# jopohl/urh

Hardware: NVIDIA H100
Metric: MSamples/s IQ demod+digitize (complex64) (higher is better)
Workload: dtype f32

## Files before the change

### urh_b200/csrc/dense_f32.cuh

```cuda
#pragma once
#include "dense.cuh"

struct SrcQad {
    static constexpr bool BINARY = false;
    template <typename T> __device__ __forceinline__ static int cls(T s, const UrhClassify& C, float) { return urh_classify((float)s, C); }
    template <typename T> __device__ __forceinline__ static void bits(T, const UrhClassify&, float, bool& nz, bool& ab) { nz = false; ab = false; }
    template <typename T> __device__ __forceinline__ static bool above(T, float) { return false; }
};
struct SrcQad2 {
    static constexpr bool BINARY = true;
    template <typename T> __device__ __forceinline__ static int cls(T s, const UrhClassify& C, float thr0) {
        const int c = ((float)s <= thr0) ? 0 : 1;
        return ((float)s == C.noise_value) ? -1 : c;
    }
    template <typename T> __device__ __forceinline__ static void bits(T s, const UrhClassify& C, float thr0, bool& nz, bool& ab) {
        nz = (float)s == C.noise_value;
        ab = !((float)s <= thr0) && !nz;
    }
    template <typename T> __device__ __forceinline__ static bool above(T s, float thr0) { return !((float)s <= thr0); }
};
struct SrcAbove {
    static constexpr bool BINARY = true;
    template <typename T> __device__ __forceinline__ static int cls(T s, const UrhClassify&, float thr0) { return (s > (T)thr0) ? 1 : 0; }
    template <typename T> __device__ __forceinline__ static void bits(T s, const UrhClassify&, float thr0, bool& nz, bool& ab) { nz = false; ab = s > (T)thr0; }
    template <typename T> __device__ __forceinline__ static bool above(T s, float thr0) { return s > (T)thr0; }
};
struct SrcCenter {
    static constexpr bool BINARY = true;
    template <typename T> __device__ __forceinline__ static int cls(T s, const UrhClassify&, float thr0) { return (s <= (T)thr0) ? 0 : 1; }
    template <typename T> __device__ __forceinline__ static void bits(T s, const UrhClassify&, float thr0, bool& nz, bool& ab) { nz = false; ab = !(s <= (T)thr0); }
    template <typename T> __device__ __forceinline__ static bool above(T s, float thr0) { return !(s <= (T)thr0); }
};

struct UrhSpec {
    const float* tg;
    float* margin;
    int64_t lo, hi;
    unsigned int* redone;
};

template <typename T> struct UrhVec2;
template <> struct UrhVec2<float> { typedef float2 type; };
template <> struct UrhVec2<double> { typedef double2 type; };

template <typename SRC, typename T>
__global__ void __launch_bounds__(URH_WARPS_PER_BLOCK * 32)
k_dense_f32(const T* __restrict__ x, int64_t n, int vec_in, const __grid_constant__ UrhClassify cls, int tol,
            UrhTileSummary* __restrict__ tiles, uint32_t* __restrict__ staging, int stage_cap,
            int16_t* __restrict__ init_cls, int cls_of_zero, const float* __restrict__ d_thr0 = nullptr,
            const UrhTileStats* __restrict__ tile_stats = nullptr, const UrhSpec spec = UrhSpec{}) {
    const float thr0 = d_thr0 ? *d_thr0 : cls.thr[0];
    if (d_thr0) cls_of_zero = (0.0f <= thr0) ? 0 : 1;
    const int lane = threadIdx.x & 31;
    const int64_t tile = (int64_t)blockIdx.x * URH_WARPS_PER_BLOCK + (threadIdx.x >> 5);
    const int64_t tile_start = tile * URH_TILE;
    if (tile_start >= n) return;
    const int tile_len = (int)((n - tile_start) < URH_TILE ? (n - tile_start) : URH_TILE);
    const int iters = (tile_len + 63) >> 6;
    if (tile_stats && tile_stats[tile].all_noise) {
        if (lane == 0) {
            UrhTileSummary s;
            s.first_cls = -1; s.last_cls = -1; s.head_len = tile_len; s.tail_len = tile_len; s.ncand = 0;
            tiles[tile] = s;
            if (tile_start == 0 && init_cls) *init_cls = (int16_t)-1;
        }
        return;
    }
    if (tile >= spec.lo && tile < spec.hi) {
        if (spec.margin[tile] > fabsf(__fsub_rn(thr0, *spec.tg))) return;
        if (lane == 0) atomicAdd(spec.redone, 1u);
    }
    UrhRunTracker rt;
    rt.init(tol, staging + tile * (int64_t)stage_cap);
    if (vec_in && tile_len == URH_TILE) {
        typedef typename UrhVec2<T>::type V;
        const V* p = (const V*)(x + tile_start) + lane;
        constexpr int ITERS = URH_TILE / 64;
        const bool no_noise = SRC::BINARY && tile_stats && cls.noise_value <= -4.0f && tile_stats[tile].cnt == URH_TILE;
        V cur[4], nxt[4];
#pragma unroll
        for (int j = 0; j < 4; j++) cur[j] = __ldg(p + j * 32);
        if (tile_start == 0 && lane == 0 && init_cls) *init_cls = (int16_t)(((float)cur[0].x == cls.noise_value) ? -1 : cls_of_zero);
        if (SRC::BINARY) {
            UrhTileResolve tr;
            tr.init();
#pragma unroll 1
            for (int it = 0; it < ITERS; it += 4) {
                if (it + 4 < ITERS) {
#pragma unroll
                    for (int j = 0; j < 4; j++) nxt[j] = __ldg(p + (it + 4 + j) * 32);
                }
                if (no_noise) {
#pragma unroll
                    for (int j = 0; j < 4; j++)
                        tr.keep(it + j, 0u, __ballot_sync(URH_FULL_MASK, SRC::template above<T>(cur[j].x, thr0)), 0u,
                                __ballot_sync(URH_FULL_MASK, SRC::template above<T>(cur[j].y, thr0)), lane);
                } else {
#pragma unroll
                    for (int j = 0; j < 4; j++) {
                        bool nx, ax, ny, ay;
                        SRC::template bits<T>(cur[j].x, cls, thr0, nx, ax);
                        SRC::template bits<T>(cur[j].y, cls, thr0, ny, ay);
                        tr.keep(it + j, __ballot_sync(URH_FULL_MASK, nx), __ballot_sync(URH_FULL_MASK, ax), __ballot_sync(URH_FULL_MASK, ny),
                                __ballot_sync(URH_FULL_MASK, ay), lane);
                    }
                }
#pragma unroll
                for (int j = 0; j < 4; j++) cur[j] = nxt[j];
            }
            tr.finish(tol, staging + tile * (int64_t)stage_cap, tiles + tile, lane);
            return;
        }
#pragma unroll 1
        for (int it = 0; it < ITERS; it += 4) {
            if (it + 4 < ITERS) {
#pragma unroll
                for (int j = 0; j < 4; j++) nxt[j] = __ldg(p + (it + 4 + j) * 32);
            }
#pragma unroll
            for (int j = 0; j < 4; j++)
                rt.feed(it + j, SRC::template cls<T>(cur[j].x, cls, thr0), SRC::template cls<T>(cur[j].y, cls, thr0), true, true, lane);
#pragma unroll
            for (int j = 0; j < 4; j++) cur[j] = nxt[j];
        }
        rt.finish(tile_len, tiles + tile, lane);
        return;
    }
    for (int it = 0; it < iters; it += 2) {
        T a0 = 0, a1 = 0, b0 = 0, b1 = 0;
        const int64_t pa = tile_start + (int64_t)it * 64 + 2 * lane;
        const int64_t pb = pa + 64;
        if (vec_in && pa + 1 < n) {
            const typename UrhVec2<T>::type v = __ldg((const typename UrhVec2<T>::type*)(x + pa));
            a0 = v.x; a1 = v.y;
        } else {
            if (pa < n) a0 = __ldg(x + pa);
            if (pa + 1 < n) a1 = __ldg(x + pa + 1);
        }
        const bool has_b = it + 1 < iters;
        if (has_b) {
            if (vec_in && pb + 1 < n) {
                const typename UrhVec2<T>::type v = __ldg((const typename UrhVec2<T>::type*)(x + pb));
                b0 = v.x; b1 = v.y;
            } else {
                if (pb < n) b0 = __ldg(x + pb);
                if (pb + 1 < n) b1 = __ldg(x + pb + 1);
            }
        }
        if (pa == 0 && init_cls) *init_cls = (int16_t)(((float)a0 == cls.noise_value) ? -1 : cls_of_zero);
        rt.feed(it, SRC::template cls<T>(a0, cls, thr0), SRC::template cls<T>(a1, cls, thr0), pa < n, pa + 1 < n, lane);
        if (has_b) rt.feed(it + 1, SRC::template cls<T>(b0, cls, thr0), SRC::template cls<T>(b1, cls, thr0), pb < n, pb + 1 < n, lane);
    }
    rt.finish(tile_len, tiles + tile, lane);
}
```

### urh_b200/csrc/digitize.cu

```cuda
#include "dense.cuh"
#include "scan.cuh"
#include "sparse.cuh"
#ifndef URH_FAST_MIN_BLOCKS
#define URH_FAST_MIN_BLOCKS 4
#endif
#include "fsk_fast.cuh"
#include "dense_f32.cuh"

#include <math.h>
#include <stdlib.h>


template <int DT, int MOD, bool DIGITIZE>
__device__ __forceinline__ void dense_iq_tile(const void* __restrict__ iq, int64_t n, const UrhDemodParams& dp, float* __restrict__ qad_out,
                                              int vec_in, int vec_out, const UrhClassify& cls, int tol, UrhTileSummary* __restrict__ tiles,
                                              uint32_t* __restrict__ staging, int stage_cap, int16_t* __restrict__ init_cls, int cls_of_zero,
                                              int64_t tile, int has_halo, UrhTileStats* __restrict__ tile_stats, const UrhFine& fine,
                                              unsigned int* s_fine, unsigned int* g_fine) {
    const int lane = threadIdx.x & 31;
    const int64_t tile_start = tile * URH_TILE;
    const int tile_len = (int)((n - tile_start) < URH_TILE ? (n - tile_start) : URH_TILE);
    const int iters = (tile_len + 63) >> 6;

    UrhRunTracker rt;
    if (DIGITIZE) rt.init(tol, staging + tile * (int64_t)stage_cap);
    UrhStatAcc acc;
    acc.init();

    float cA = 0.0f, cB = 0.0f;
    if (MOD == URH_MOD_FSK && (tile_start > 0 || has_halo) && lane == 0) {
        typedef typename UrhElem<DT>::type E;
        const E* pp = (const E*)iq + 2 * (tile_start - 1);
        const UrhFskTerms t = urh_fsk_terms((float)pp[0], (float)pp[1]);
        cA = t.A; cB = t.B;
    }

    UrhPair cur = urh_load_pair<DT>(iq, tile_start + 2 * lane, n, vec_in != 0);
    for (int it = 0; it < iters; it++) {
        const int64_t pos0 = tile_start + (int64_t)it * 64 + 2 * lane;
        UrhPair nxt;
        if (it + 1 < iters) nxt = urh_load_pair<DT>(iq, pos0 + 64, n, vec_in != 0);

        const float m0 = __fadd_rn(__fmul_rn(cur.r0, cur.r0), __fmul_rn(cur.i0, cur.i0));
        const float m1 = __fadd_rn(__fmul_rn(cur.r1, cur.r1), __fmul_rn(cur.i1, cur.i1));
        float s0 = dp.noise_value, s1 = dp.noise_value;
        if (MOD == URH_MOD_FSK) {
            const UrhFskTerms t0 = urh_fsk_terms(cur.r0, cur.i0);
            const UrhFskTerms t1 = urh_fsk_terms(cur.r1, cur.i1);
            float pA = __shfl_up_sync(URH_FULL_MASK, t1.A, 1);
            float pB = __shfl_up_sync(URH_FULL_MASK, t1.B, 1);
            if (lane == 0) { pA = cA; pB = cB; }
            cA = __shfl_sync(URH_FULL_MASK, t1.A, 31);
            cB = __shfl_sync(URH_FULL_MASK, t1.B, 31);
            if (!(m0 <= dp.noise_sqrd)) s0 = urh_fsk_angle(pA, pB, t0.C, t0.D);
            if (!(m1 <= dp.noise_sqrd)) s1 = urh_fsk_angle(t0.A, t0.B, t1.C, t1.D);
        } else if (MOD == URH_MOD_ASK) {
            if (!(m0 <= dp.noise_sqrd)) s0 = __fdiv_rn(__fsqrt_rn(m0), dp.max_mag);
            if (!(m1 <= dp.noise_sqrd)) s1 = __fdiv_rn(__fsqrt_rn(m1), dp.max_mag);
        }
        if (pos0 == 0 && !has_halo) s0 = dp.noise_value;

        const bool v0 = pos0 < n, v1 = pos0 + 1 < n;
        if (tile_stats) {
            if (v0) { acc.add(s0); acc.all_noise = acc.all_noise && (s0 == dp.noise_value); }
            if (v1) { acc.add(s1); acc.all_noise = acc.all_noise && (s1 == dp.noise_value); }
            if (s_fine) {
                if (v0) urh_fine_add(s0, fine, s_fine, g_fine);
                if (v1) urh_fine_add(s1, fine, s_fine, g_fine);
            }
        }
        if (qad_out) {
            if (v1 && vec_out) urh_stg_f2(qad_out + pos0, s0, s1);
            else {
                if (v0) qad_out[pos0] = s0;
                if (v1) qad_out[pos0 + 1] = s1;
            }
        }
        if (DIGITIZE) {
            const int c0 = urh_classify(s0, cls), c1 = urh_classify(s1, cls);
            if (pos0 == 0) *init_cls = (int16_t)((s0 == cls.noise_value) ? -1 : cls_of_zero);
            rt.feed(it, c0, c1, v0, v1, lane);
        }
        cur = nxt;
    }
    if (tile_stats) acc.store(tile_stats + tile, lane);
    if (DIGITIZE) rt.finish(tile_len, tiles + tile, lane);
}

template <int DT, int MOD, bool DIGITIZE>
__global__ void __launch_bounds__(URH_WARPS_PER_BLOCK * 32)
k_dense_iq(const void* __restrict__ iq, int64_t n, UrhDemodParams dp, float* __restrict__ qad_out, int vec_in,
           int vec_out, const __grid_constant__ UrhClassify cls, int tol, UrhTileSummary* __restrict__ tiles,
           uint32_t* __restrict__ staging, int stage_cap, int16_t* __restrict__ init_cls, int cls_of_zero,
           int64_t tile_begin, int64_t tile_count, int has_halo, UrhTileStats* __restrict__ tile_stats, const UrhFine fine) {
    extern __shared__ unsigned int s_fine[];
    const int64_t tile_rel = (int64_t)blockIdx.x * URH_WARPS_PER_BLOCK + (threadIdx.x >> 5);
    const int64_t block_tile0 = tile_begin + (int64_t)blockIdx.x * URH_WARPS_PER_BLOCK;
    if (fine.gh) urh_fine_zero(s_fine);
    if (tile_rel < tile_count && (tile_begin + tile_rel) * URH_TILE < n)
        dense_iq_tile<DT, MOD, DIGITIZE>(iq, n, dp, qad_out, vec_in, vec_out, cls, tol, tiles, staging, stage_cap, init_cls, cls_of_zero,
                                    tile_begin + tile_rel, has_halo, tile_stats, fine,
                                    fine.gh ? s_fine : nullptr, fine.gh ? urh_fine_row(fine, tile_begin + tile_rel, block_tile0) : nullptr);
    if (fine.gh) urh_fine_flush(fine, s_fine, block_tile0);
}

template <int DT, bool DIGITIZE, bool WRITE, bool STATS>
__global__ void __launch_bounds__(URH_WARPS_PER_BLOCK * 32, URH_FAST_MIN_BLOCKS)
k_fsk_fast(const void* __restrict__ iq, int64_t n, UrhDemodParams dp, float* __restrict__ qad_out, float thr0,
           float cls_noise, int tol, UrhTileSummary* __restrict__ tiles, uint32_t* __restrict__ staging, int stage_cap,
           int64_t tile_begin, int64_t tile_count, UrhTileStats* __restrict__ tile_stats, const UrhFine fine) {
    extern __shared__ unsigned int s_fine[];
    const bool fine_on = STATS && fine.gh;
    const int lane = threadIdx.x & 31;
    const int64_t tile_rel = (int64_t)blockIdx.x * URH_WARPS_PER_BLOCK + (threadIdx.x >> 5);
    const int64_t block_tile0 = tile_begin + (int64_t)blockIdx.x * URH_WARPS_PER_BLOCK;
    if (fine_on) urh_fine_zero(s_fine);
    if (tile_rel < tile_count) {
        const int64_t tile = tile_begin + tile_rel;
        UrhRunTracker rt;
        if (DIGITIZE) rt.init(tol, staging + tile * (int64_t)stage_cap);
        UrhOne one;
        one.p = dp.one;
        one.m = dp.mone;
        urh_fsk_full_tile<DT, DIGITIZE, WRITE, STATS>(iq, n, tile * URH_TILE, dp, qad_out, thr0, cls_noise, rt, lane, one,
                                                      STATS ? tile_stats + tile : nullptr, 0u, DIGITIZE ? tiles + tile : nullptr, fine,
                                                      fine_on ? s_fine : nullptr, fine_on ? urh_fine_row(fine, tile, block_tile0) : nullptr);
    }
    if (fine_on) urh_fine_flush(fine, s_fine, block_tile0);
}

#define URH_FSK_FIFO 3
template <int DT, bool DIGITIZE, bool WRITE, bool STATS>
__global__ void __launch_bounds__(URH_WARPS_PER_BLOCK * 32, (DT == URH_DT_F32) ? 5 : 4)
k_fsk_fifo(const void* __restrict__ iq, int64_t n, UrhDemodParams dp, float* __restrict__ qad_out, float thr0,
           float cls_noise, int tol, UrhTileSummary* __restrict__ tiles, uint32_t* __restrict__ staging, int stage_cap,
           int64_t tile_begin, int64_t tile_count, UrhTileStats* __restrict__ tile_stats, const UrhFine fine,
           const float* __restrict__ d_thr0 = nullptr, float* __restrict__ margin = nullptr) {
    __shared__ __align__(16) unsigned char s_fifo[URH_WARPS_PER_BLOCK][URH_FSK_FIFO + 1][64 * 2 * sizeof(typename UrhElem<DT>::type)];
    extern __shared__ unsigned int s_fine[];
    const bool fine_on = STATS && fine.gh;
    if (DIGITIZE && STATS) thr0 = *d_thr0;
    const int lane = threadIdx.x & 31;
    const int64_t tile_rel = (int64_t)blockIdx.x * URH_WARPS_PER_BLOCK + (threadIdx.x >> 5);
    const int64_t block_tile0 = tile_begin + (int64_t)blockIdx.x * URH_WARPS_PER_BLOCK;
    if (fine_on) urh_fine_zero(s_fine);
    if (tile_rel < tile_count) {
        const int64_t tile = tile_begin + tile_rel;
        UrhRunTracker rt;
        if (DIGITIZE) rt.init(tol, staging + tile * (int64_t)stage_cap);
        UrhOne one;
        one.p = dp.one;
        one.m = dp.mone;
        const uint32_t fifo = (uint32_t)__cvta_generic_to_shared(&s_fifo[threadIdx.x >> 5][0][0]);
        urh_fsk_full_tile<DT, DIGITIZE, WRITE, STATS, URH_FSK_FIFO>(iq, n, tile * URH_TILE, dp, qad_out, thr0, cls_noise, rt, lane, one,
                                                                    STATS ? tile_stats + tile : nullptr, fifo,
                                                                    DIGITIZE ? tiles + tile : nullptr, fine, fine_on ? s_fine : nullptr,
                                                                    fine_on ? urh_fine_row(fine, tile, block_tile0) : nullptr,
                                                                    (DIGITIZE && STATS) ? margin + tile : nullptr);
    }
    if (fine_on) urh_fine_flush(fine, s_fine, block_tile0);
}

#define URH_GUESS_SAMPLES 16384
#define URH_GUESS_BINS 128
#define URH_GUESS_THREADS 1024
__global__ void __launch_bounds__(URH_GUESS_THREADS) k_speculate_guess(const float2* __restrict__ iq, int64_t n, float noise_sqrd, int forced,
                                                                      float forced_tg, float* __restrict__ d_tg, unsigned int* __restrict__ redone) {
    constexpr int PER = URH_GUESS_SAMPLES / URH_GUESS_THREADS;
    __shared__ unsigned int s_hist[URH_GUESS_BINS];
    __shared__ float s_mn[32], s_mx[32];
    if (forced) {
        if (threadIdx.x == 0) { *d_tg = forced_tg; *redone = 0u; }
        return;
    }
    for (int b = threadIdx.x; b < URH_GUESS_BINS; b += blockDim.x) s_hist[b] = 0u;
    float v[PER];
    float mn = INFINITY, mx = -INFINITY;
#pragma unroll
    for (int k = 0; k < PER; k++) {
        const int64_t i = 1 + (int64_t)(k * URH_GUESS_THREADS + threadIdx.x) * (n - 1) / URH_GUESS_SAMPLES;
        const float2 p = iq[i - 1], c = iq[i];
        v[k] = NAN;
        if (!(c.x * c.x + c.y * c.y <= noise_sqrd)) {
            v[k] = atan2f(p.x * c.y - p.y * c.x, p.x * c.x + p.y * c.y);
            mn = fminf(mn, v[k]);
            mx = fmaxf(mx, v[k]);
        }
    }
    for (int off = 16; off > 0; off >>= 1) {
        mn = fminf(mn, __shfl_xor_sync(URH_FULL_MASK, mn, off));
        mx = fmaxf(mx, __shfl_xor_sync(URH_FULL_MASK, mx, off));
    }
    if ((threadIdx.x & 31) == 0) { s_mn[threadIdx.x >> 5] = mn; s_mx[threadIdx.x >> 5] = mx; }
    __syncthreads();
    mn = INFINITY; mx = -INFINITY;
    for (int w = 0; w < URH_GUESS_THREADS / 32; w++) { mn = fminf(mn, s_mn[w]); mx = fmaxf(mx, s_mx[w]); }
    const float width = (mx - mn) / URH_GUESS_BINS;
    if (width > 0.0f) {
#pragma unroll
        for (int k = 0; k < PER; k++)
            if (!isnan(v[k])) atomicAdd(&s_hist[min((int)((v[k] - mn) / width), URH_GUESS_BINS - 1)], 1u);
    }
    __syncthreads();
    if (threadIdx.x != 0) return;
    *redone = 0u;
    if (!(mn <= mx)) { *d_tg = 0.0f; return; }
    if (!(width > 0.0f)) { *d_tg = mn; return; }
    constexpr int WINDOW = (int)(0.05 * URH_GUESS_BINS) + 1;
    int top[2] = {-1, -1};
    for (int b = 0; b < URH_GUESS_BINS; b++) {
        const unsigned int y = s_hist[b];
        bool peak = y > 0u;
        for (int d = 1; d < WINDOW && peak; d++)
            peak = y > (b + d < URH_GUESS_BINS ? s_hist[b + d] : 0u) && y > (b - d >= 0 ? s_hist[b - d] : 0u);
        if (!peak) continue;
        if (top[0] < 0 || y > s_hist[top[0]]) { top[1] = top[0]; top[0] = b; }
        else if (top[1] < 0 || y > s_hist[top[1]]) top[1] = b;
    }
    if (top[0] < 0) *d_tg = 0.5f * (mn + mx);
    else if (top[1] < 0) *d_tg = mn + ((float)top[0] + 0.5f) * width;
    else *d_tg = mn + (0.5f * (float)(top[0] + top[1]) + 0.5f) * width;
}


extern "C" int urh_get_center_thresholds(float center, float spacing, int modulation_order, float* h_out) {
    const int n = modulation_order / 2;
    for (int i = 0; i < n; i++) {
        volatile float t = (float)(n - (i + 1)) * spacing;
        h_out[i] = center - t;
    }
    for (int i = n; i < modulation_order - 1; i++) {
        volatile float t = (float)(i + 1 - n) * spacing;
        h_out[i] = center + t;
    }
    return URH_OK;
}

static int fill_classify(urh_ctx* ctx, UrhClassify* C, int mod_type, float center, uint8_t bits_per_symbol,
                         float spacing) {
    if (bits_per_symbol > 8) URH_FAIL(ctx, URH_ERR_INVALID, "bits_per_symbol %d > 8 not supported", (int)bits_per_symbol);
    memset(C, 0, sizeof(*C));
    C->noise_value = urh_noise_value(mod_type);
    C->order = 1 << bits_per_symbol;
    if (C->order > 1) urh_get_center_thresholds(center, spacing, C->order, C->thr);
    return URH_OK;
}

static int host_classify(float s, const UrhClassify& C) {
    int c = C.order - 1;
    for (int k = 0; k < C.order - 1; k++)
        if (s <= C.thr[k]) { c = k; break; }
    return c;
}

static float max_magnitude_for(int dtype) {
    switch (dtype) {
        case URH_DT_I8: return (float)sqrt(127.0 * 127.0 + 128.0 * 128.0);
        case URH_DT_U8: return (float)sqrt(255.0 * 255.0);
        case URH_DT_I16: return (float)sqrt(32768.0 * 32768.0 + 32767.0 * 32767.0);
        case URH_DT_U16: return (float)sqrt(65535.0 * 65535.0);
        default: return (float)sqrt(2.0);
    }
}

static bool iq_vec_aligned(const void* p, int dtype) { return ((uintptr_t)p % (2 * (size_t)urh_iq_bytes(dtype))) == 0; }

template <int DT, int MOD, bool DIG>
static int launch_dense_iq_t(urh_ctx* ctx, const void* d_iq, int64_t n, const UrhDemodParams& dp, float* d_qad,
                             const UrhClassify& cls, int tol, UrhTileSummary* tiles, uint32_t* staging,
                             int stage_cap, int16_t* init_cls, int cls_of_zero, int has_halo = 0,
                             UrhTileStats* tile_stats = nullptr, int64_t tile_lo = 0, int64_t tile_hi = -1,
                             const UrhFine& fine = UrhFine{}, UrhSpec* spec = nullptr) {
    const int64_t ntiles = urh_div_up(n, URH_TILE);
    const size_t fine_smem = fine.gh ? (size_t)URH_FINE_NB * sizeof(unsigned int) : 0;
    if (tile_hi < 0 || tile_hi > ntiles) tile_hi = ntiles;
    const int vec_in = iq_vec_aligned(d_iq, DT) ? 1 : 0;
    const int vec_out = (d_qad && ((uintptr_t)d_qad % 8) == 0) ? 1 : 0;
    const int threads = URH_WARPS_PER_BLOCK * 32;
    auto generic = [&](int64_t begin, int64_t end) -> int {
        begin = begin < tile_lo ? tile_lo : begin;
        end = end > tile_hi ? tile_hi : end;
        const int64_t count = end - begin;
        if (count <= 0) return URH_OK;
        URH_LAUNCH(ctx, (k_dense_iq<DT, MOD, DIG>), (unsigned)urh_div_up(count, URH_WARPS_PER_BLOCK), threads, fine_smem, d_iq, n, dp,
                   d_qad, vec_in, vec_out, cls, tol, tiles, staging, stage_cap, init_cls, cls_of_zero, begin, count, has_halo,
                   tile_stats, fine);
        return URH_OK;
    };
    const int64_t nfull = n / URH_TILE;
    const bool fast = MOD == URH_MOD_FSK && vec_in && (!d_qad || vec_out) && (!DIG || cls.order == 2) && nfull > 1;
    URH_PROF_BEGIN(ctx);
    if (fast) {
        const int64_t fb = tile_lo > 1 ? tile_lo : 1, fe = tile_hi < nfull ? tile_hi : nfull;
        if (fe > fb) {
            const unsigned grid = (unsigned)urh_div_up(fe - fb, URH_WARPS_PER_BLOCK);
            static const bool fifo = getenv("URH_B200_FSK_NO_FIFO") == nullptr;
            const bool ff = fifo;
            bool speculated = false;
            if constexpr (DT == URH_DT_F32 && MOD == URH_MOD_FSK && !DIG) {
                if (spec && ff && tile_stats && d_qad) {
                    URH_LAUNCH(ctx, (k_fsk_fifo<DT, true, true, true>), grid, threads, fine_smem, d_iq, n, dp, d_qad, 0.0f, dp.noise_value,
                               tol, tiles, staging, stage_cap, fb, fe - fb, tile_stats, fine, (const float*)spec->tg, spec->margin);
                    spec->lo = fb;
                    spec->hi = fe;
                    speculated = true;
                }
            }
            if (speculated) {
            } else if (tile_stats && d_qad && !DIG) {
                if (ff) URH_LAUNCH(ctx, (k_fsk_fifo<DT, false, true, true>), grid, threads, fine_smem, d_iq, n, dp, d_qad, cls.thr[0], cls.noise_value,
                                   tol, tiles, staging, stage_cap, fb, fe - fb, tile_stats, fine);
                else URH_LAUNCH(ctx, (k_fsk_fast<DT, false, true, true>), grid, threads, fine_smem, d_iq, n, dp, d_qad, cls.thr[0], cls.noise_value,
                                tol, tiles, staging, stage_cap, fb, fe - fb, tile_stats, fine);
            } else if (d_qad) {
                if (ff) URH_LAUNCH(ctx, (k_fsk_fifo<DT, DIG, true, false>), grid, threads, 0, d_iq, n, dp, d_qad, cls.thr[0], cls.noise_value, tol,
                                   tiles, staging, stage_cap, fb, fe - fb, nullptr, UrhFine{});
                else URH_LAUNCH(ctx, (k_fsk_fast<DT, DIG, true, false>), grid, threads, 0, d_iq, n, dp, d_qad, cls.thr[0], cls.noise_value, tol,
                                tiles, staging, stage_cap, fb, fe - fb, nullptr, UrhFine{});
            } else {
                if (ff) URH_LAUNCH(ctx, (k_fsk_fifo<DT, DIG, false, false>), grid, threads, 0, d_iq, n, dp, d_qad, cls.thr[0], cls.noise_value, tol,
                                   tiles, staging, stage_cap, fb, fe - fb, nullptr, UrhFine{});
                else URH_LAUNCH(ctx, (k_fsk_fast<DT, DIG, false, false>), grid, threads, 0, d_iq, n, dp, d_qad, cls.thr[0], cls.noise_value, tol,
                                tiles, staging, stage_cap, fb, fe - fb, nullptr, UrhFine{});
            }
        }
        URH_CHECK(generic(0, 1));
        URH_CHECK(generic(nfull, ntiles));
    } else {
        URH_CHECK(generic(0, ntiles));
    }
    URH_PROF_END(ctx);
    return URH_OK;
}

template <int MOD, bool DIG>
static int launch_dense_iq_m(urh_ctx* ctx, int dtype, const void* d_iq, int64_t n, const UrhDemodParams& dp,
                             float* d_qad, const UrhClassify& cls, int tol, UrhTileSummary* tiles,
                             uint32_t* staging, int stage_cap, int16_t* init_cls, int cls_of_zero, int has_halo = 0,
                             UrhTileStats* tile_stats = nullptr, int64_t tile_lo = 0, int64_t tile_hi = -1,
                             const UrhFine& fine = UrhFine{}, UrhSpec* spec = nullptr) {
    switch (dtype) {
        case URH_DT_I8: return launch_dense_iq_t<URH_DT_I8, MOD, DIG>(ctx, d_iq, n, dp, d_qad, cls, tol, tiles, staging, stage_cap, init_cls, cls_of_zero, has_halo, tile_stats, tile_lo, tile_hi, fine);
        case URH_DT_U8: return launch_dense_iq_t<URH_DT_U8, MOD, DIG>(ctx, d_iq, n, dp, d_qad, cls, tol, tiles, staging, stage_cap, init_cls, cls_of_zero, has_halo, tile_stats, tile_lo, tile_hi, fine);
        case URH_DT_I16: return launch_dense_iq_t<URH_DT_I16, MOD, DIG>(ctx, d_iq, n, dp, d_qad, cls, tol, tiles, staging, stage_cap, init_cls, cls_of_zero, has_halo, tile_stats, tile_lo, tile_hi, fine);
        case URH_DT_U16: return launch_dense_iq_t<URH_DT_U16, MOD, DIG>(ctx, d_iq, n, dp, d_qad, cls, tol, tiles, staging, stage_cap, init_cls, cls_of_zero, has_halo, tile_stats, tile_lo, tile_hi, fine);
        case URH_DT_F32: return launch_dense_iq_t<URH_DT_F32, MOD, DIG>(ctx, d_iq, n, dp, d_qad, cls, tol, tiles, staging, stage_cap, init_cls, cls_of_zero, has_halo, tile_stats, tile_lo, tile_hi, fine, spec);
        default: URH_FAIL(ctx, URH_ERR_DTYPE, "Unsupported dtype");
    }
}

int urh_costas_demod(urh_ctx* ctx, const void* d_iq, int dtype, int64_t n, float noise_sqrd, int loop_order,
                     float bandwidth, float* d_out);

static UrhDemodParams make_demod_params(float noise_mag, int mod_type, int dtype) {
    UrhDemodParams dp;
    volatile float nm = noise_mag;
    volatile float sq = nm * nm;
    dp.noise_sqrd = sq;
    dp.noise_value = urh_noise_value(mod_type);
    dp.max_mag = max_magnitude_for(dtype);
    dp.one = 1.0f;
    dp.mone = -1.0f;
    return dp;
}

extern "C" int urh_afp_demod(urh_ctx* ctx, const void* d_iq, int dtype, int64_t n, float noise_mag, int mod_type,
                             int mod_order, float costas_loop_bandwidth, float* d_out) {
    if (n < 0) URH_FAIL(ctx, URH_ERR_INVALID, "negative length");
    if (urh_iq_bytes(dtype) == 0) URH_FAIL(ctx, URH_ERR_DTYPE, "Unsupported dtype");
    if (n == 0) return URH_OK;
    if (n <= 2 || (mod_type != URH_MOD_ASK && mod_type != URH_MOD_FSK && mod_type != URH_MOD_PSK)) {
        URH_CUDA(ctx, cudaMemsetAsync(d_out, 0, (size_t)n * sizeof(float), ctx->stream));
        if (n > 2) {
            const float nv = urh_noise_value(mod_type);
            URH_CUDA(ctx, cudaMemcpyAsync(d_out, &nv, sizeof(float), cudaMemcpyHostToDevice, ctx->stream));
            URH_CUDA(ctx, cudaStreamSynchronize(ctx->stream));
        }
        return URH_OK;
    }
    const UrhDemodParams dp = make_demod_params(noise_mag, mod_type, dtype);
    if (mod_type == URH_MOD_PSK) return urh_costas_demod(ctx, d_iq, dtype, n, dp.noise_sqrd, mod_order, costas_loop_bandwidth, d_out);
    UrhClassify cls;
    memset(&cls, 0, sizeof(cls));
    if (mod_type == URH_MOD_ASK)
        return launch_dense_iq_m<URH_MOD_ASK, false>(ctx, dtype, d_iq, n, dp, d_out, cls, 0, nullptr, nullptr, 0, nullptr, 0);
    return launch_dense_iq_m<URH_MOD_FSK, false>(ctx, dtype, d_iq, n, dp, d_out, cls, 0, nullptr, nullptr, 0, nullptr, 0);
}

int urh_center_tiles_begin(urh_ctx* ctx, const float* d_x, const UrhTileStats* ts, int64_t n, int64_t* h_total);

extern "C" int urh_afp_demod_tiles(urh_ctx* ctx, const void* d_iq, int dtype, int64_t n, float noise_mag, int mod_type,
                                   float* d_qad_out, int halo, int64_t* h_kept) {
    if (n <= 2 || (mod_type != URH_MOD_ASK && mod_type != URH_MOD_FSK) || !d_qad_out)
        URH_FAIL(ctx, URH_ERR_INVALID, "urh_afp_demod_tiles: ASK/FSK, n > 2 and a qad buffer are required");
    if (urh_iq_bytes(dtype) == 0) URH_FAIL(ctx, URH_ERR_DTYPE, "Unsupported dtype");
    urh_arena_reset(ctx);
    const UrhDemodParams dp = make_demod_params(noise_mag, mod_type, dtype);
    UrhClassify cls;
    memset(&cls, 0, sizeof(cls));
    const int64_t ntiles = urh_div_up(n, URH_TILE);
    UrhTileStats* ts;
    URH_CHECK(urh_arena(ctx, (size_t)ntiles, &ts));
    if (mod_type == URH_MOD_ASK)
        URH_CHECK((launch_dense_iq_m<URH_MOD_ASK, false>(ctx, dtype, d_iq, n, dp, d_qad_out, cls, 0, nullptr, nullptr, 0, nullptr, 0, halo, ts)));
    else
        URH_CHECK((launch_dense_iq_m<URH_MOD_FSK, false>(ctx, dtype, d_iq, n, dp, d_qad_out, cls, 0, nullptr, nullptr, 0, nullptr, 0, halo, ts)));
    return urh_center_tiles_begin(ctx, d_qad_out, ts, n, h_kept);
}

int urh_finish_local(urh_ctx* ctx, int64_t n, int tol, bool is_ask, uint32_t sps, const UrhTileSummary* tiles, const uint32_t* staging,
                     int stage_cap, const int16_t* d_init, int64_t* k);
int urh_finish_shard(urh_ctx* ctx, int64_t n, int tol, bool is_ask, uint32_t sps, const UrhTileSummary* tiles, const uint32_t* staging,
                     int stage_cap, const int16_t* d_init, int64_t global_offset, int64_t n_total, int64_t* k);

static int digitize_finish(urh_ctx* ctx, int64_t n, int tol, bool is_ask, uint32_t sps, UrhTileSummary* tiles,
                           uint32_t* staging, int stage_cap, int16_t* d_init, int64_t* k) {
    if (getenv("URH_B200_OLD_FINISH")) {
        UrhCandidates cand;
        URH_CHECK(urh_collect_candidates(ctx, n, tol, tiles, staging, stage_cap, &cand));
        return urh_pulses_from_candidates(ctx, n, tol, is_ask, sps, cand, d_init, k);
    }
    return urh_finish_local(ctx, n, tol, is_ask, sps, tiles, staging, stage_cap, d_init, k);
}

static int stage_cap_for(int tol) { return URH_TILE / (tol + 1) + 2; }

extern "C" int urh_grab_pulse_lens(urh_ctx* ctx, const float* d_qad, int64_t n, float center, uint16_t tolerance,
                                   int mod_type, uint32_t samples_per_symbol, uint8_t bits_per_symbol,
                                   float center_spacing, int64_t* k) {
    if (!k) return URH_ERR_INVALID;
    *k = 0;
    ctx->pulses_k = 0;
    if (n < 0) URH_FAIL(ctx, URH_ERR_INVALID, "negative length");
    if (n == 0) return URH_OK;
    urh_arena_reset(ctx);
    UrhClassify cls;
    URH_CHECK(fill_classify(ctx, &cls, mod_type, center, bits_per_symbol, center_spacing));
    const int tol = tolerance;
    const int64_t ntiles = urh_div_up(n, URH_TILE);
    const int cap = stage_cap_for(tol);
    UrhTileSummary* tiles;
    uint32_t* staging;
    int16_t* d_init;
    URH_CHECK(urh_arena(ctx, (size_t)ntiles, &tiles));
    URH_CHECK(urh_arena(ctx, (size_t)ntiles * cap, &staging));
    URH_CHECK(urh_arena(ctx, 8, &d_init));
    const unsigned grid = (unsigned)urh_div_up(ntiles, URH_WARPS_PER_BLOCK);
    const int vec_in = (((uintptr_t)d_qad % 8) == 0) ? 1 : 0;
    URH_PROF_BEGIN(ctx);
    if (cls.order == 2)
        URH_LAUNCH(ctx, (k_dense_f32<SrcQad2, float>), grid, URH_WARPS_PER_BLOCK * 32, 0, d_qad, n, vec_in, cls, tol, tiles,
                   staging, cap, d_init, host_classify(0.0f, cls));
    else
        URH_LAUNCH(ctx, (k_dense_f32<SrcQad, float>), grid, URH_WARPS_PER_BLOCK * 32, 0, d_qad, n, vec_in, cls, tol, tiles,
                   staging, cap, d_init, host_classify(0.0f, cls));
    URH_PROF_END(ctx);
    return digitize_finish(ctx, n, tol, mod_type == URH_MOD_ASK, samples_per_symbol, tiles, staging, cap, d_init, k);
}

extern "C" int urh_demod_digitize(urh_ctx* ctx, const void* d_iq, int dtype, int64_t n, float noise_mag,
                                  int mod_type, float center, uint16_t tolerance, uint32_t samples_per_symbol,
                                  uint8_t bits_per_symbol, float center_spacing, float* d_qad_out, int64_t* k) {
    if (!k) return URH_ERR_INVALID;
    *k = 0;
    ctx->pulses_k = 0;
    if (n < 0) URH_FAIL(ctx, URH_ERR_INVALID, "negative length");
    if (urh_iq_bytes(dtype) == 0) URH_FAIL(ctx, URH_ERR_DTYPE, "Unsupported dtype");
    if (n == 0) return URH_OK;
    if (n <= 2 || (mod_type != URH_MOD_ASK && mod_type != URH_MOD_FSK)) {
        float* q = d_qad_out;
        if (!q) URH_CUDA(ctx, cudaMalloc((void**)&q, (size_t)n * sizeof(float)));
        int rc = urh_afp_demod(ctx, d_iq, dtype, n, noise_mag, mod_type, 1 << bits_per_symbol, 0.1f, q);
        if (rc == URH_OK)
            rc = urh_grab_pulse_lens(ctx, q, n, center, tolerance, mod_type, samples_per_symbol, bits_per_symbol,
                                     center_spacing, k);
        if (!d_qad_out) {
            cudaStreamSynchronize(ctx->stream);
            cudaFree(q);
        }
        return rc;
    }
    urh_arena_reset(ctx);
    UrhClassify cls;
    URH_CHECK(fill_classify(ctx, &cls, mod_type, center, bits_per_symbol, center_spacing));
    const UrhDemodParams dp = make_demod_params(noise_mag, mod_type, dtype);
    const int tol = tolerance;
    const int64_t ntiles = urh_div_up(n, URH_TILE);
    const int cap = stage_cap_for(tol);
    UrhTileSummary* tiles;
    uint32_t* staging;
    int16_t* d_init;
    URH_CHECK(urh_arena(ctx, (size_t)ntiles, &tiles));
    URH_CHECK(urh_arena(ctx, (size_t)ntiles * cap, &staging));
    URH_CHECK(urh_arena(ctx, 8, &d_init));
    const int c0 = host_classify(0.0f, cls);
    if (mod_type == URH_MOD_ASK)
        URH_CHECK((launch_dense_iq_m<URH_MOD_ASK, true>(ctx, dtype, d_iq, n, dp, d_qad_out, cls, tol, tiles, staging, cap, d_init, c0)));
    else
        URH_CHECK((launch_dense_iq_m<URH_MOD_FSK, true>(ctx, dtype, d_iq, n, dp, d_qad_out, cls, tol, tiles, staging, cap, d_init, c0)));
    return digitize_finish(ctx, n, tol, mod_type == URH_MOD_ASK, samples_per_symbol, tiles, staging, cap, d_init, k);
}

extern "C" int urh_shard_dense(urh_ctx* ctx, const void* d_iq, int dtype, int64_t n, int has_halo, float noise_mag, int mod_type,
                               float center, uint16_t tolerance, uint8_t bits_per_symbol, float center_spacing,
                               float* d_qad_out, int64_t* h_summary) {
    if (n <= 0) URH_FAIL(ctx, URH_ERR_INVALID, "empty shard");
    if (mod_type != URH_MOD_ASK && mod_type != URH_MOD_FSK) URH_FAIL(ctx, URH_ERR_INVALID, "sharded path: ASK / FSK only (PSK is a serial recurrence)");
    if (urh_iq_bytes(dtype) == 0) URH_FAIL(ctx, URH_ERR_DTYPE, "Unsupported dtype");
    urh_arena_reset(ctx);
    UrhClassify cls;
    URH_CHECK(fill_classify(ctx, &cls, mod_type, center, bits_per_symbol, center_spacing));
    const UrhDemodParams dp = make_demod_params(noise_mag, mod_type, dtype);
    const int tol = tolerance;
    const int64_t ntiles = urh_div_up(n, URH_TILE);
    const int cap = stage_cap_for(tol);
    UrhTileSummary* tiles;
    uint32_t* staging;
    int16_t* d_init;
    URH_CHECK(urh_arena(ctx, (size_t)ntiles, &tiles));
    URH_CHECK(urh_arena(ctx, (size_t)ntiles * cap, &staging));
    URH_CHECK(urh_arena(ctx, 8, &d_init));
    URH_CUDA(ctx, cudaMemsetAsync(d_init, 0, 16, ctx->stream));
    const int c0 = host_classify(0.0f, cls);
    if (mod_type == URH_MOD_ASK)
        URH_CHECK((launch_dense_iq_m<URH_MOD_ASK, true>(ctx, dtype, d_iq, n, dp, d_qad_out, cls, tol, tiles, staging, cap, d_init, c0, has_halo)));
    else
        URH_CHECK((launch_dense_iq_m<URH_MOD_FSK, true>(ctx, dtype, d_iq, n, dp, d_qad_out, cls, tol, tiles, staging, cap, d_init, c0, has_halo)));
    ctx->shard_tiles = tiles;
    ctx->shard_staging = staging;
    ctx->shard_cap = cap;
    ctx->shard_n = n;
    ctx->shard_tol = tol;
    URH_CHECK(urh_shard_run_total(ctx, n, tiles, h_summary));
    int16_t init16 = 0;
    URH_CUDA(ctx, cudaMemcpyAsync(&init16, d_init, sizeof(int16_t), cudaMemcpyDeviceToHost, ctx->stream));
    URH_CUDA(ctx, cudaStreamSynchronize(ctx->stream));
    h_summary[3] = init16;
    return URH_OK;
}

extern "C" int urh_shard_dense_qad(urh_ctx* ctx, const float* d_qad, int64_t n, int mod_type, float center, uint16_t tolerance,
                                   uint8_t bits_per_symbol, float center_spacing, int64_t* h_summary) {
    if (n <= 0) URH_FAIL(ctx, URH_ERR_INVALID, "empty shard");
    urh_arena_reset(ctx);
    UrhClassify cls;
    URH_CHECK(fill_classify(ctx, &cls, mod_type, center, bits_per_symbol, center_spacing));
    const int tol = tolerance;
    const int64_t ntiles = urh_div_up(n, URH_TILE);
    const int cap = stage_cap_for(tol);
    UrhTileSummary* tiles;
    uint32_t* staging;
    int16_t* d_init;
    URH_CHECK(urh_arena(ctx, (size_t)ntiles, &tiles));
    URH_CHECK(urh_arena(ctx, (size_t)ntiles * cap, &staging));
    URH_CHECK(urh_arena(ctx, 8, &d_init));
    URH_CUDA(ctx, cudaMemsetAsync(d_init, 0, 16, ctx->stream));
    const int vec_in = (((uintptr_t)d_qad % 8) == 0) ? 1 : 0;
    URH_PROF_BEGIN(ctx);
    const unsigned grid = (unsigned)urh_div_up(ntiles, URH_WARPS_PER_BLOCK);
    if (cls.order == 2)
        URH_LAUNCH(ctx, (k_dense_f32<SrcQad2, float>), grid, URH_WARPS_PER_BLOCK * 32, 0, d_qad, n, vec_in, cls, tol, tiles, staging, cap,
                   d_init, host_classify(0.0f, cls));
    else
        URH_LAUNCH(ctx, (k_dense_f32<SrcQad, float>), grid, URH_WARPS_PER_BLOCK * 32, 0, d_qad, n, vec_in, cls, tol, tiles, staging, cap,
                   d_init, host_classify(0.0f, cls));
    URH_PROF_END(ctx);
    ctx->shard_tiles = tiles;
    ctx->shard_staging = staging;
    ctx->shard_cap = cap;
    ctx->shard_n = n;
    ctx->shard_tol = tol;
    URH_CHECK(urh_shard_run_total(ctx, n, tiles, h_summary));
    int16_t init16 = 0;
    URH_CUDA(ctx, cudaMemcpyAsync(&init16, d_init, sizeof(int16_t), cudaMemcpyDeviceToHost, ctx->stream));
    URH_CUDA(ctx, cudaStreamSynchronize(ctx->stream));
    h_summary[3] = init16;
    return URH_OK;
}

int urh_finish_chunk(urh_ctx* ctx, int64_t n, int tol, bool is_ask, uint32_t sps, const UrhTileSummary* tiles, const uint32_t* staging,
                     int stage_cap, const int16_t* d_init, UrhChain* chain, int64_t global_offset, int64_t n_total, int64_t row_base,
                     int64_t rows_cap, int64_t* k);

#define URH_STREAM_MAX_RING 8
#define URH_STREAM_PAD 256
enum { URH_OP_UPLOAD = 0, URH_OP_COMPUTE = 1, URH_OP_DOWNLOAD = 2 };

static int64_t stream_chunk_samples(int64_t n, int64_t cs) {
    if (cs <= 0) cs = (int64_t)1 << 24;
    cs -= cs % URH_TILE;
    if (cs < URH_TILE) cs = URH_TILE;
    const int64_t whole = urh_div_up(n > 0 ? n : 1, URH_TILE) * URH_TILE;
    return cs < whole ? cs : whole;
}
static int64_t rows_bound(int64_t n, int tol) { return n / (tol + 1) + 3; }

extern "C" int urh_stream_schedule(int64_t n, int64_t chunk_samples, int ring, int flags, int64_t* h_ops, int64_t cap, int64_t* count) {
    if (!count || n < 0 || ring < 2 || ring > URH_STREAM_MAX_RING) return URH_ERR_INVALID;
    const int64_t cs = stream_chunk_samples(n, chunk_samples);
    const int64_t chunks = urh_div_up(n, cs);
    const bool up = flags & URH_STREAM_UPLOAD, down = flags & URH_STREAM_DOWNLOAD, halo = flags & URH_STREAM_HALO;
    int64_t k = 0;
    auto emit = [&](int64_t kind, int64_t c) {
        if (h_ops && k < cap) {
            int64_t* o = h_ops + 6 * k;
            o[0] = kind; o[1] = c; o[2] = c % ring; o[3] = c * cs; o[4] = (c + 1) * cs < n ? (c + 1) * cs : n;
            o[5] = (kind == URH_OP_UPLOAD && halo && c > 0) ? 1 : 0;
        }
        k++;
    };
    if (up)
        for (int64_t c = 0; c < ring - 1 && c < chunks; c++) emit(URH_OP_UPLOAD, c);
    for (int64_t c = 0; c < chunks; c++) {
        if (up && c + ring - 1 < chunks) emit(URH_OP_UPLOAD, c + ring - 1);
        emit(URH_OP_COMPUTE, c);
        if (down) emit(URH_OP_DOWNLOAD, c);
    }
    *count = k;
    return (h_ops && k > cap) ? URH_ERR_INVALID : URH_OK;
}

struct StreamSizes {
    int64_t cs;
    int64_t src_slot;
    int64_t qad_slot;
    int64_t ring_bytes;
    int64_t arena;
    int64_t scan_items;
    int64_t rows_chunk;
};
static int64_t r256(int64_t b) { return (b + 255) & ~(int64_t)255; }
static int64_t finish_arena_bytes(int64_t tiles, int64_t rows_cap, bool ask) {
    return r256(tiles * (int64_t)sizeof(RunCarry)) + 2 * r256(tiles * 4) + 2 * r256(tiles * 8) + r256((32 + 8) * 8) +
           (ask ? r256(rows_cap * 16) : 0);
}
static int psk_order_of(int entry) { return (entry & URH_STREAM_PSK) ? ((entry & URH_STREAM_PSK4) ? 4 : 2) : 0; }
static int psk_entry_flags(int mod_order) { return URH_STREAM_PSK | (mod_order >= 4 ? URH_STREAM_PSK4 : 0); }

static StreamSizes stream_sizes(int64_t n, int dtype, int tol, int64_t chunk_samples, int ring, int entry) {
    StreamSizes z;
    const int kind = entry & 0xf;
    const int psk = psk_order_of(entry);
    const bool resident = entry & URH_STREAM_RESIDENT;
    const int64_t ntiles = urh_div_up(n, URH_TILE);
    z.cs = resident ? ntiles * URH_TILE : stream_chunk_samples(n, chunk_samples);
    const int64_t ct = z.cs / URH_TILE;
    const int64_t cap = stage_cap_for(tol);
    const bool iq = kind != URH_STREAM_ENTRY_GRAB_PULSE_LENS;
    const bool digitize = kind != URH_STREAM_ENTRY_AFP_DEMOD;
    z.rows_chunk = rows_bound(z.cs, tol);
    if (resident) {
        z.src_slot = iq ? n * urh_iq_bytes(dtype) : n * 4;
        z.qad_slot = (kind == URH_STREAM_ENTRY_GRAB_PULSE_LENS) ? 0 : n * 4;
        z.ring_bytes = r256(z.src_slot) + r256(z.qad_slot);
    } else {
        z.src_slot = (kind == URH_STREAM_ENTRY_GRAB_PULSE_LENS && (entry & URH_STREAM_QAD_ON_DEVICE)) ? 0
                     : URH_STREAM_PAD + z.cs * (iq ? urh_iq_bytes(dtype) : 4);
        const bool qad_ring = kind == URH_STREAM_ENTRY_AFP_DEMOD ||
                              (kind == URH_STREAM_ENTRY_DEMOD_DIGITIZE && ((entry & URH_STREAM_QAD_OUT) || psk));
        z.qad_slot = qad_ring ? z.cs * 4 : 0;
        z.ring_bytes = ring * (r256(z.src_slot) + r256(z.qad_slot));
        if (kind == URH_STREAM_ENTRY_DEMOD_CENTER_DIGITIZE) z.ring_bytes += r256(n * 4);
    }
    z.arena = 0;
    z.scan_items = ct > z.rows_chunk ? ct : z.rows_chunk;
    if (digitize) z.arena += r256(ct * (int64_t)sizeof(UrhTileSummary)) + r256(ct * cap * 4) + r256(16) + r256(sizeof(UrhChain)) +
                             finish_arena_bytes(ct, z.rows_chunk, true);
    if (psk && !resident) z.arena += urh_costas_arena_bytes(z.cs, psk) + r256(16) + r256(6 * 8);
    if (kind == URH_STREAM_ENTRY_DEMOD_CENTER_DIGITIZE) {
        z.arena += r256(ntiles * (int64_t)sizeof(UrhTileStats)) + r256((int64_t)URH_FINE_SLABS * URH_FINE_NB * 4) + r256((ntiles + 1) * 8) +
                   ((int64_t)2 << 20);
        if (ntiles > z.scan_items) z.scan_items = ntiles;
    }
    return z;
}

extern "C" int urh_stream_footprint(int64_t n, int dtype, int tolerance, int64_t chunk_samples, int ring, int entry, int64_t rows,
                                    int64_t* bytes) {
    if (!bytes || n < 0 || tolerance < 0 || tolerance > 0xffff || (entry & 0xf) > URH_STREAM_ENTRY_DEMOD_CENTER_DIGITIZE) return URH_ERR_INVALID;
    if (!(entry & URH_STREAM_RESIDENT) && (ring < 2 || ring > URH_STREAM_MAX_RING)) return URH_ERR_INVALID;
    if ((entry & 0xf) != URH_STREAM_ENTRY_GRAB_PULSE_LENS && urh_iq_bytes(dtype) == 0) return URH_ERR_DTYPE;
    if ((entry & URH_STREAM_PSK) && (entry & 0xf) != URH_STREAM_ENTRY_AFP_DEMOD && (entry & 0xf) != URH_STREAM_ENTRY_DEMOD_DIGITIZE)
        return URH_ERR_INVALID;
    const StreamSizes z = stream_sizes(n, dtype, tolerance, chunk_samples, ring, entry);
    const bool digitize = (entry & 0xf) != URH_STREAM_ENTRY_AFP_DEMOD;
    const int64_t r = rows == -2 ? n / 64 + 1024 : (rows < 0 ? rows_bound(n, tolerance) : rows);
    if (entry & URH_STREAM_RESIDENT) {
        const int64_t ntiles = urh_div_up(n, URH_TILE);
        int64_t b = z.ring_bytes + ((int64_t)64 << 20);
        if (digitize)
            b += r256(ntiles * (int64_t)sizeof(UrhTileSummary)) + r256(ntiles * (int64_t)stage_cap_for(tolerance) * 4) +
                 finish_arena_bytes(ntiles, r + r / 4, true) + 16 * (r + r / 4);
        if ((entry & 0xf) == URH_STREAM_ENTRY_DEMOD_CENTER_DIGITIZE)
            b += r256(ntiles * (int64_t)sizeof(UrhTileStats)) + r256((int64_t)URH_FINE_SLABS * URH_FINE_NB * 4) + r256((ntiles + 1) * 8);
        if (psk_order_of(entry)) b += urh_costas_arena_bytes(n, psk_order_of(entry));
        *bytes = b;
        return URH_OK;
    }
    int64_t b = z.ring_bytes;
    b += 2 * z.arena + ((int64_t)64 << 20);
    const int64_t nb = 2 * (z.scan_items / 256 + 1);
    b += 256 + (nb > 8192 ? nb : 8192) * (4 + 2 * 32);
    if (digitize) b += 3 * 16 * (r + z.rows_chunk);
    *bytes = b;
    return URH_OK;
}

extern "C" int urh_stream_stats(urh_ctx* ctx, int64_t* h_out3) {
    h_out3[0] = ctx->stream_free_low;
    h_out3[1] = ctx->stream_chunks;
    h_out3[2] = (int64_t)ctx->arena_peak;
    return URH_OK;
}

struct StreamRing {
    urh_ctx* ctx = nullptr;
    char* mem = nullptr;
    cudaEvent_t ev[3][URH_STREAM_MAX_RING] = {};
    int ring = 0;
    int init(urh_ctx* c, int r, int64_t bytes) {
        ctx = c;
        ring = r;
        ctx->stream_free_low = -1;
        for (int k = 0; k < 3; k++)
            for (int s = 0; s < r; s++) URH_CUDA(ctx, cudaEventCreateWithFlags(&ev[k][s], cudaEventDisableTiming));
        if (bytes > 0) URH_CUDA(ctx, cudaMallocAsync((void**)&mem, (size_t)bytes, ctx->stream));
        URH_CUDA(ctx, cudaEventRecord(ctx->ev_comp[0], ctx->stream));
        URH_CUDA(ctx, cudaStreamWaitEvent(ctx->copy_stream[0], ctx->ev_comp[0], 0));
        URH_CUDA(ctx, cudaStreamWaitEvent(ctx->copy_stream[1], ctx->ev_comp[0], 0));
        return URH_OK;
    }
    ~StreamRing() {
        if (!ctx) return;
        cudaStreamSynchronize(ctx->copy_stream[0]);
        cudaStreamSynchronize(ctx->copy_stream[1]);
        if (mem) cudaFreeAsync(mem, ctx->stream);
        cudaStreamSynchronize(ctx->stream);
        for (int k = 0; k < 3; k++)
            for (int s = 0; s < ring; s++)
                if (ev[k][s]) cudaEventDestroy(ev[k][s]);
    }
};

template <typename F>
static int stream_run(urh_ctx* ctx, int64_t n, int64_t cs, StreamRing& R, const char* h_src, int src_b, bool halo, char* d_src,
                      int64_t src_slot, float* h_qad, float* d_qad, F&& compute, bool qad_resident = false) {
    const int flags = (h_src ? URH_STREAM_UPLOAD : 0) | (h_qad ? URH_STREAM_DOWNLOAD : 0) | (halo ? URH_STREAM_HALO : 0);
    int64_t count = 0;
    URH_CHECK(urh_stream_schedule(n, cs, R.ring, flags, nullptr, 0, &count));
    std::vector<int64_t> ops((size_t)(6 * count));
    URH_CHECK(urh_stream_schedule(n, cs, R.ring, flags, ops.data(), count, &count));
    bool recorded[3][URH_STREAM_MAX_RING] = {};
    ctx->stream_chunks = 0;
    for (int64_t i = 0; i < count; i++) {
        const int64_t* o = &ops[(size_t)(6 * i)];
        const int kind = (int)o[0], s = (int)o[2];
        const int64_t c = o[1], s0 = o[3], s1 = o[4], h = o[5];
        if (kind == URH_OP_UPLOAD) {
            cudaStream_t cp = ctx->copy_stream[0];
            if (recorded[URH_OP_COMPUTE][s]) URH_CUDA(ctx, cudaStreamWaitEvent(cp, R.ev[URH_OP_COMPUTE][s], 0));
            URH_CUDA(ctx, cudaMemcpyAsync(d_src + s * src_slot + URH_STREAM_PAD - h * src_b, h_src + (s0 - h) * src_b,
                                          (size_t)((s1 - s0 + h) * src_b), cudaMemcpyHostToDevice, cp));
            URH_CUDA(ctx, cudaEventRecord(R.ev[URH_OP_UPLOAD][s], cp));
        } else if (kind == URH_OP_COMPUTE) {
            if (h_src) URH_CUDA(ctx, cudaStreamWaitEvent(ctx->stream, R.ev[URH_OP_UPLOAD][s], 0));
            if (h_qad && !qad_resident && recorded[URH_OP_DOWNLOAD][s])
                URH_CUDA(ctx, cudaStreamWaitEvent(ctx->stream, R.ev[URH_OP_DOWNLOAD][s], 0));
            URH_CHECK(compute(c, s0, s1, s));
            URH_CUDA(ctx, cudaEventRecord(R.ev[URH_OP_COMPUTE][s], ctx->stream));
            urh_stream_sample_free(ctx);
            ctx->stream_chunks++;
        } else {
            cudaStream_t cp = ctx->copy_stream[1];
            URH_CUDA(ctx, cudaStreamWaitEvent(cp, R.ev[URH_OP_COMPUTE][s], 0));
            URH_CUDA(ctx, cudaMemcpyAsync(h_qad + s0, d_qad + (qad_resident ? s0 : (int64_t)s * cs), (size_t)(s1 - s0) * sizeof(float),
                                          cudaMemcpyDeviceToHost, cp));
            URH_CUDA(ctx, cudaEventRecord(R.ev[URH_OP_DOWNLOAD][s], cp));
        }
        recorded[kind][s] = true;
    }
    URH_CUDA(ctx, cudaStreamSynchronize(ctx->copy_stream[1]));
    URH_CUDA(ctx, cudaStreamSynchronize(ctx->stream));
    return URH_OK;
}

struct StreamDigitizer {
    UrhTileSummary* tiles;
    uint32_t* staging;
    int16_t* d_init;
    UrhChain* chain;
    int cap, tol;
    bool is_ask;
    uint32_t sps;
    int64_t n, rows, rows_all;
    UrhArenaMark mark;
    int init(urh_ctx* ctx, int64_t n_total, int64_t cs, int tolerance, bool ask, uint32_t samples_per_symbol) {
        n = n_total; tol = tolerance; is_ask = ask; sps = samples_per_symbol; rows = 0;
        cap = stage_cap_for(tol);
        rows_all = rows_bound(n, tol);
        const int64_t ct = cs / URH_TILE;
        URH_CHECK(urh_arena(ctx, (size_t)ct, &tiles));
        URH_CHECK(urh_arena(ctx, (size_t)ct * cap, &staging));
        URH_CHECK(urh_arena(ctx, 8, &d_init));
        URH_CHECK(urh_arena(ctx, 1, &chain));
        URH_CUDA(ctx, cudaMemsetAsync(d_init, 0, 16, ctx->stream));
        mark = urh_arena_mark(ctx);
        return URH_OK;
    }
    int finish(urh_ctx* ctx, int64_t s0, int64_t s1) {
        const int64_t rc = rows_bound(s1 - s0, tol);
        const int64_t need = rows + rc;
        if (need > (int64_t)ctx->pulses_cap_rows) {
            int64_t grow = 2 * (int64_t)ctx->pulses_cap_rows;
            if (grow > rows_all + rc) grow = rows_all + rc;
            URH_CHECK(urh_ensure_pulses_keep(ctx, (size_t)(grow > need ? grow : need), (size_t)rows));
        }
        urh_arena_release(ctx, mark);
        int64_t kc = 0;
        URH_CHECK(urh_finish_chunk(ctx, s1 - s0, tol, is_ask, sps, tiles, staging, cap, d_init, chain, s0, n, rows, rc, &kc));
        urh_stream_sample_free(ctx);
        rows += kc;
        return URH_OK;
    }
};

static int stream_check(urh_ctx* ctx, int64_t n, int ring, int mod_type, int dtype, bool iq);
static int psk_stream_check(urh_ctx* ctx, int64_t n, int ring, int dtype) {
    URH_CHECK(stream_check(ctx, n, ring, URH_MOD_PSK, dtype, false));
    if (n <= 2) URH_FAIL(ctx, URH_ERR_INVALID, "streamed PSK demodulation: n > 2");
    if (urh_iq_bytes(dtype) == 0) URH_FAIL(ctx, URH_ERR_DTYPE, "Unsupported dtype");
    return URH_OK;
}

static int stream_check(urh_ctx* ctx, int64_t n, int ring, int mod_type, int dtype, bool iq) {
    if (n <= 0) URH_FAIL(ctx, URH_ERR_INVALID, "streamed call: empty capture");
    if (ring < 2 || ring > URH_STREAM_MAX_RING) URH_FAIL(ctx, URH_ERR_INVALID, "streamed call: ring of %d slots (2..%d)", ring, URH_STREAM_MAX_RING);
    if (iq && (n <= 2 || (mod_type != URH_MOD_ASK && mod_type != URH_MOD_FSK)))
        URH_FAIL(ctx, URH_ERR_INVALID, "streamed demodulation: ASK/FSK and n > 2 (PSK is a serial recurrence)");
    if (iq && urh_iq_bytes(dtype) == 0) URH_FAIL(ctx, URH_ERR_DTYPE, "Unsupported dtype");
    return URH_OK;
}

template <bool DIG>
static int stream_dense_iq(urh_ctx* ctx, int dtype, int mod_type, const char* d_src, int64_t src_slot, int64_t n, const UrhDemodParams& dp,
                           float* qad_global, const UrhClassify& cls, int tol, StreamDigitizer* dz, int64_t s0, int64_t s1, int s,
                           UrhTileStats* ts = nullptr, const UrhFine& fine = UrhFine{}) {
    const int b = urh_iq_bytes(dtype);
    const void* iq = d_src + s * src_slot + URH_STREAM_PAD - s0 * b;
    const int64_t t0 = s0 / URH_TILE, t1 = urh_div_up(s1, URH_TILE);
    UrhTileSummary* tiles = dz ? dz->tiles - t0 : nullptr;
    uint32_t* staging = dz ? dz->staging - t0 * dz->cap : nullptr;
    const int cap = dz ? dz->cap : 0;
    int16_t* init = dz ? dz->d_init : nullptr;
    const int c0 = DIG ? host_classify(0.0f, cls) : 0;
    if (mod_type == URH_MOD_ASK)
        return launch_dense_iq_m<URH_MOD_ASK, DIG>(ctx, dtype, iq, n, dp, qad_global, cls, tol, tiles, staging, cap, init, c0, 0, ts, t0, t1, fine);
    return launch_dense_iq_m<URH_MOD_FSK, DIG>(ctx, dtype, iq, n, dp, qad_global, cls, tol, tiles, staging, cap, init, c0, 0, ts, t0, t1, fine);
}

static int stream_dense_qad(urh_ctx* ctx, const float* x, int64_t s0, int64_t s1, const UrhClassify& cls, StreamDigitizer& dz,
                            const float* d_thr0 = nullptr, const UrhTileStats* ts = nullptr) {
    const int64_t nc = s1 - s0;
    const unsigned grid = (unsigned)urh_div_up(urh_div_up(nc, URH_TILE), URH_WARPS_PER_BLOCK);
    const int vec_in = (((uintptr_t)x % 8) == 0) ? 1 : 0;
    int16_t* init = s0 == 0 ? dz.d_init : nullptr;
    const int c0 = d_thr0 ? 0 : host_classify(0.0f, cls);
    const UrhTileStats* tsc = ts ? ts + s0 / URH_TILE : nullptr;
    if (cls.order == 2)
        URH_LAUNCH(ctx, (k_dense_f32<SrcQad2, float>), grid, URH_WARPS_PER_BLOCK * 32, 0, x, nc, vec_in, cls, dz.tol, dz.tiles, dz.staging,
                   dz.cap, init, c0, d_thr0, tsc);
    else
        URH_LAUNCH(ctx, (k_dense_f32<SrcQad, float>), grid, URH_WARPS_PER_BLOCK * 32, 0, x, nc, vec_in, cls, dz.tol, dz.tiles, dz.staging,
                   dz.cap, init, c0, d_thr0, tsc);
    return URH_OK;
}

struct CenterPlan;
int urh_center_chain(urh_ctx* ctx, const float* d_qad, int64_t n, const UrhTileStats* ts, int64_t max_size, int rank, int world,
                     const UrhFine* fine, CenterPlan** d_plan_out);
int urh_center_plan_result(urh_ctx* ctx, const CenterPlan* plan, const float** d_centerf, const double** d_center, const int** d_state);
int urh_center_plan_certify_stats(urh_ctx* ctx, const CenterPlan* plan, int64_t* h_dst3);

extern "C" int urh_shard_digitize(urh_ctx* ctx, const void* d_iq, int dtype, const float* d_qad_in, int64_t n, int has_halo,
                                  float noise_mag, int mod_type, float center, uint16_t tolerance, uint32_t samples_per_symbol,
                                  uint8_t bits_per_symbol, float center_spacing, float* d_qad_out, int64_t global_offset,
                                  int64_t n_total, int64_t* k) {
    if (!k) return URH_ERR_INVALID;
    *k = 0;
    ctx->pulses_k = 0;
    if (n <= 0) URH_FAIL(ctx, URH_ERR_INVALID, "empty shard");
    if (mod_type != URH_MOD_ASK && mod_type != URH_MOD_FSK) URH_FAIL(ctx, URH_ERR_INVALID, "sharded path: ASK / FSK only");
    if (!d_qad_in && urh_iq_bytes(dtype) == 0) URH_FAIL(ctx, URH_ERR_DTYPE, "Unsupported dtype");
    if (!ctx->nccl_comm) URH_FAIL(ctx, URH_ERR_INVALID, "NCCL communicator not initialised (urh_nccl_init)");
    urh_arena_reset(ctx);
    UrhClassify cls;
    URH_CHECK(fill_classify(ctx, &cls, mod_type, center, bits_per_symbol, center_spacing));
    const int tol = tolerance;
    const int64_t ntiles = urh_div_up(n, URH_TILE);
    const int cap = stage_cap_for(tol);
    UrhTileSummary* tiles;
    uint32_t* staging;
    int16_t* d_init;
    URH_CHECK(urh_arena(ctx, (size_t)ntiles, &tiles));
    URH_CHECK(urh_arena(ctx, (size_t)ntiles * cap, &staging));
    URH_CHECK(urh_arena(ctx, 8, &d_init));
    URH_CUDA(ctx, cudaMemsetAsync(d_init, 0, 16, ctx->stream));
    const int c0 = host_classify(0.0f, cls);
    if (d_qad_in) {
        const int vec_in = (((uintptr_t)d_qad_in % 8) == 0) ? 1 : 0;
        const unsigned grid = (unsigned)urh_div_up(ntiles, URH_WARPS_PER_BLOCK);
        URH_PROF_BEGIN(ctx);
        if (cls.order == 2)
            URH_LAUNCH(ctx, (k_dense_f32<SrcQad2, float>), grid, URH_WARPS_PER_BLOCK * 32, 0, d_qad_in, n, vec_in, cls, tol, tiles, staging, cap,
                       d_init, c0, (const float*)nullptr);
        else
            URH_LAUNCH(ctx, (k_dense_f32<SrcQad, float>), grid, URH_WARPS_PER_BLOCK * 32, 0, d_qad_in, n, vec_in, cls, tol, tiles, staging, cap,
                       d_init, c0, (const float*)nullptr);
        URH_PROF_END(ctx);
    } else {
        const UrhDemodParams dp = make_demod_params(noise_mag, mod_type, dtype);
        if (mod_type == URH_MOD_ASK)
            URH_CHECK((launch_dense_iq_m<URH_MOD_ASK, true>(ctx, dtype, d_iq, n, dp, d_qad_out, cls, tol, tiles, staging, cap, d_init, c0, has_halo)));
        else
            URH_CHECK((launch_dense_iq_m<URH_MOD_FSK, true>(ctx, dtype, d_iq, n, dp, d_qad_out, cls, tol, tiles, staging, cap, d_init, c0, has_halo)));
    }
    return urh_finish_shard(ctx, n, tol, mod_type == URH_MOD_ASK, samples_per_symbol, tiles, staging, cap, d_init, global_offset, n_total, k);
}

struct StreamCenter {
    int ring;
    int64_t chunk_samples;
    const void* h_iq;
    float* h_qad;
    int64_t* kept;
};
static int demod_center_digitize_impl(urh_ctx* ctx, const void* d_iq, int dtype, int64_t n, int has_halo, float noise_mag, int mod_type,
                                      uint16_t tolerance, uint32_t samples_per_symbol, int64_t max_size, float* d_qad_out, bool sharded,
                                      int64_t global_offset, int64_t n_total, double* center, int* center_state, int64_t* k,
                                      const void* h_iq = nullptr, int64_t chunk_samples = 0, const StreamCenter* sc = nullptr) {
    if (!k || !center || !center_state) return URH_ERR_INVALID;
    *k = 0;
    *center = 0.0;
    *center_state = 0;
    ctx->pulses_k = 0;
    if (n <= 2 || (mod_type != URH_MOD_ASK && mod_type != URH_MOD_FSK) || !d_qad_out)
        URH_FAIL(ctx, URH_ERR_INVALID, "demod_center_digitize: ASK/FSK, n > 2 and a qad buffer are required");
    if (urh_iq_bytes(dtype) == 0) URH_FAIL(ctx, URH_ERR_DTYPE, "Unsupported dtype");
    if (sharded && !ctx->nccl_comm) URH_FAIL(ctx, URH_ERR_INVALID, "NCCL communicator not initialised (urh_nccl_init)");
    urh_arena_reset(ctx);
    URH_TL_RESET(ctx);
    URH_TL_MARK(ctx, "step start");
    const UrhDemodParams dp = make_demod_params(noise_mag, mod_type, dtype);
    UrhClassify cls;
    memset(&cls, 0, sizeof(cls));
    const int64_t ntiles = urh_div_up(n, URH_TILE);
    UrhTileStats* ts;
    URH_CHECK(urh_arena(ctx, (size_t)ntiles, &ts));
    const bool no_certify = getenv("URH_B200_CENTER_NO_CERTIFY") != nullptr;
    UrhFine fine = {};
    if (!sharded && !no_certify) {
        fine.slab_tiles = urh_div_up(ntiles, URH_FINE_SLABS);
        if (fine.slab_tiles < URH_WARPS_PER_BLOCK) fine.slab_tiles = URH_WARPS_PER_BLOCK;
        const int64_t nslabs = urh_div_up(ntiles, fine.slab_tiles);
        URH_CHECK(urh_arena(ctx, (size_t)(nslabs * URH_FINE_NB), &fine.gh));
        URH_CUDA(ctx, cudaMemsetAsync(fine.gh, 0, (size_t)(nslabs * URH_FINE_NB) * sizeof(unsigned int), ctx->stream));
        fine.scale = (mod_type == URH_MOD_FSK) ? 512.0f : 4096.0f;
        fine.off = (mod_type == URH_MOD_FSK) ? 2048.0f : 0.0f;
    }
    const int64_t chunk_tiles = (h_iq && chunk_samples > 0) ? (chunk_samples >= URH_TILE ? chunk_samples / URH_TILE : 1) : ntiles;
    const size_t sample_bytes = (size_t)urh_iq_bytes(dtype);
    StreamRing ring;
    int64_t scs = 0;
    if (sc) {
        const StreamSizes z = stream_sizes(n, dtype, tolerance, sc->chunk_samples, sc->ring, URH_STREAM_ENTRY_DEMOD_CENTER_DIGITIZE);
        scs = z.cs;
        URH_CHECK(ring.init(ctx, sc->ring, sc->ring * r256(z.src_slot)));
        const int64_t slot = r256(z.src_slot);
        URH_CHECK(stream_run(ctx, n, scs, ring, (const char*)sc->h_iq, urh_iq_bytes(dtype), true, ring.mem, slot, sc->h_qad, d_qad_out,
                             [&](int64_t, int64_t s0, int64_t s1, int s) {
                                 return stream_dense_iq<false>(ctx, dtype, mod_type, ring.mem, slot, n, dp, d_qad_out, cls, 0, nullptr, s0, s1, s,
                                                               ts, fine);
                             }, true));
    }
    cls.noise_value = urh_noise_value(mod_type);
    cls.order = 2;
    const int tol = tolerance;
    const int cap = stage_cap_for(tol);
    UrhTileSummary* tiles = nullptr;
    uint32_t* staging = nullptr;
    int16_t* d_init = nullptr;
    if (!sc) {
        URH_CHECK(urh_arena(ctx, (size_t)ntiles, &tiles));
        URH_CHECK(urh_arena(ctx, (size_t)ntiles * cap, &staging));
        URH_CHECK(urh_arena(ctx, 8, &d_init));
    }
    const bool speculate = !sharded && !h_iq && !sc && mod_type == URH_MOD_FSK && dtype == URH_DT_F32 &&
                           getenv("URH_B200_NO_SPECULATE") == nullptr;
    UrhSpec spec = {};
    if (speculate) {
        float* tg;
        URH_CHECK(urh_arena(ctx, 1, &tg));
        URH_CHECK(urh_arena(ctx, 1, &spec.redone));
        URH_CHECK(urh_arena(ctx, (size_t)ntiles, &spec.margin));
        spec.tg = tg;
        const char* forced = getenv("URH_B200_SPECULATE_GUESS");
        URH_LAUNCH(ctx, k_speculate_guess, 1, URH_GUESS_THREADS, 0, (const float2*)d_iq, n, dp.noise_sqrd, forced ? 1 : 0,
                   forced ? strtof(forced, nullptr) : 0.0f, tg, spec.redone);
    }
    int chunk_no = 0;
    for (int64_t t0 = 0; t0 < (sc ? 0 : ntiles); t0 += chunk_tiles, chunk_no++) {
        const int64_t t1 = (t0 + chunk_tiles < ntiles) ? t0 + chunk_tiles : ntiles;
        if (h_iq) {
            const int64_t s0 = t0 * URH_TILE, s1 = (t1 * URH_TILE < n) ? t1 * URH_TILE : n;
            cudaEvent_t ev = ctx->ev_copy[chunk_no & 1];
            URH_CUDA(ctx, cudaMemcpyAsync((char*)d_iq + (size_t)s0 * sample_bytes, (const char*)h_iq + (size_t)s0 * sample_bytes,
                                          (size_t)(s1 - s0) * sample_bytes, cudaMemcpyHostToDevice, ctx->copy_stream[0]));
            URH_CUDA(ctx, cudaEventRecord(ev, ctx->copy_stream[0]));
            URH_CUDA(ctx, cudaStreamWaitEvent(ctx->stream, ev, 0));
        }
        if (mod_type == URH_MOD_ASK)
            URH_CHECK((launch_dense_iq_m<URH_MOD_ASK, false>(ctx, dtype, d_iq, n, dp, d_qad_out, cls, 0, nullptr, nullptr, 0, nullptr, 0, has_halo, ts, t0, t1, fine)));
        else
            URH_CHECK((launch_dense_iq_m<URH_MOD_FSK, false>(ctx, dtype, d_iq, n, dp, d_qad_out, cls, tol, tiles, staging, cap, nullptr, 0, has_halo,
                                                             ts, t0, t1, fine, speculate ? &spec : nullptr)));
    }
    CenterPlan* plan = nullptr;
    URH_CHECK(urh_center_chain(ctx, d_qad_out, n, ts, max_size, sharded ? ctx->nccl_rank : 0, sharded ? ctx->nccl_world : 1,
                               fine.gh ? &fine : nullptr, &plan));
    const float* d_centerf;
    const double* d_center;
    const int* d_state;
    urh_center_plan_result(ctx, plan, &d_centerf, &d_center, &d_state);
    int64_t rows = 0;
    if (sc) {
        URH_CUDA(ctx, cudaMemcpyAsync(ctx->h_mail + 40, d_center, sizeof(double), cudaMemcpyDeviceToHost, ctx->stream));
        URH_CUDA(ctx, cudaMemcpyAsync(ctx->h_mail + 41, d_state, sizeof(int), cudaMemcpyDeviceToHost, ctx->stream));
        URH_CHECK(urh_center_plan_certify_stats(ctx, plan, ctx->h_mail + 42));
        URH_CUDA(ctx, cudaMemcpyAsync(ctx->h_mail + 45, (const int64_t*)ctx->center_prefix + ntiles, sizeof(int64_t), cudaMemcpyDeviceToHost,
                                      ctx->stream));
        URH_CUDA(ctx, cudaStreamSynchronize(ctx->stream));
        int st0 = 0;
        memcpy(&st0, ctx->h_mail + 41, sizeof(int));
        if (st0 == 1) {
            StreamDigitizer dz;
            URH_CHECK(dz.init(ctx, n, scs, tol, mod_type == URH_MOD_ASK, samples_per_symbol));
            for (int64_t s0 = 0; s0 < n; s0 += scs) {
                const int64_t s1 = s0 + scs < n ? s0 + scs : n;
                URH_CHECK(stream_dense_qad(ctx, d_qad_out + s0, s0, s1, cls, dz, d_centerf, ts));
                URH_CHECK(dz.finish(ctx, s0, s1));
            }
            rows = dz.rows;
        }
        *sc->kept = ctx->h_mail[45];
    } else {
        URH_CUDA(ctx, cudaMemsetAsync(d_init, 0, 16, ctx->stream));
        const int vec_in = (((uintptr_t)d_qad_out % 8) == 0) ? 1 : 0;
        URH_LAUNCH(ctx, (k_dense_f32<SrcQad2, float>), (unsigned)urh_div_up(ntiles, URH_WARPS_PER_BLOCK), URH_WARPS_PER_BLOCK * 32, 0,
                   (const float*)d_qad_out, n, vec_in, cls, tol, tiles, staging, cap, d_init, 0, d_centerf, (const UrhTileStats*)ts, spec);
        URH_CUDA(ctx, cudaMemcpyAsync(ctx->h_mail + 40, d_center, sizeof(double), cudaMemcpyDeviceToHost, ctx->stream));
        URH_CUDA(ctx, cudaMemcpyAsync(ctx->h_mail + 41, d_state, sizeof(int), cudaMemcpyDeviceToHost, ctx->stream));
        URH_CHECK(urh_center_plan_certify_stats(ctx, plan, ctx->h_mail + 42));
        ctx->h_mail[46] = 0;
        if (speculate) URH_CUDA(ctx, cudaMemcpyAsync(ctx->h_mail + 46, spec.redone, sizeof(unsigned int), cudaMemcpyDeviceToHost, ctx->stream));
        if (sharded)
            URH_CHECK(urh_finish_shard(ctx, n, tol, mod_type == URH_MOD_ASK, samples_per_symbol, tiles, staging, cap, d_init, global_offset, n_total, &rows));
        else
            URH_CHECK(urh_finish_local(ctx, n, tol, mod_type == URH_MOD_ASK, samples_per_symbol, tiles, staging, cap, d_init, &rows));
    }
    memcpy(center, ctx->h_mail + 40, sizeof(double));
    int st = 0;
    memcpy(&st, ctx->h_mail + 41, sizeof(int));
    *center_state = st;
    ctx->center_cert[0] = ctx->h_mail[42];
    ctx->center_cert[1] = fine.gh ? URH_FINE_NB : 0;
    ctx->center_cert[2] = ctx->h_mail[44];
    const int64_t redone = (spec.hi > spec.lo) ? ctx->h_mail[46] : 0;
    ctx->spec_stats[0] = spec.hi - spec.lo;
    ctx->spec_stats[1] = spec.hi - spec.lo - redone;
    ctx->spec_stats[2] = redone;
    if (st != 1) {
        ctx->pulses_k = 0;
        rows = 0;
    }
    *k = rows;
    return URH_OK;
}

extern "C" int urh_speculate_stats(urh_ctx* ctx, int64_t* h_out3) {
    for (int i = 0; i < 3; i++) h_out3[i] = ctx->spec_stats[i];
    return URH_OK;
}

extern "C" int urh_demod_center_digitize(urh_ctx* ctx, const void* d_iq, int dtype, int64_t n, float noise_mag, int mod_type,
                                         uint16_t tolerance, uint32_t samples_per_symbol, int64_t max_size, float* d_qad_out,
                                         double* center, int* center_state, int64_t* k) {
    return demod_center_digitize_impl(ctx, d_iq, dtype, n, 0, noise_mag, mod_type, tolerance, samples_per_symbol, max_size, d_qad_out, false,
                                      0, n, center, center_state, k);
}

extern "C" int urh_demod_center_digitize_host(urh_ctx* ctx, const void* h_iq, int dtype, int64_t n, float noise_mag, int mod_type,
                                              uint16_t tolerance, uint32_t samples_per_symbol, int64_t max_size, int64_t chunk_samples,
                                              void* d_iq_scratch, float* d_qad_out, double* center, int* center_state, int64_t* k) {
    if (!h_iq || !d_iq_scratch) return URH_ERR_INVALID;
    URH_CUDA(ctx, cudaEventRecord(ctx->ev_comp[0], ctx->stream));
    URH_CUDA(ctx, cudaStreamWaitEvent(ctx->copy_stream[0], ctx->ev_comp[0], 0));
    return demod_center_digitize_impl(ctx, d_iq_scratch, dtype, n, 0, noise_mag, mod_type, tolerance, samples_per_symbol, max_size, d_qad_out,
                                      false, 0, n, center, center_state, k, h_iq, chunk_samples > 0 ? chunk_samples : ((int64_t)1 << 24));
}

extern "C" int urh_shard_demod_center_digitize_host(urh_ctx* ctx, const void* h_iq, int dtype, int64_t n, int has_halo, float noise_mag,
                                                    int mod_type, uint16_t tolerance, uint32_t samples_per_symbol, int64_t max_size,
                                                    int64_t chunk_samples, void* d_iq_scratch, float* d_qad_out, int64_t global_offset,
                                                    int64_t n_total, double* center, int* center_state, int64_t* k) {
    if (!h_iq || !d_iq_scratch) return URH_ERR_INVALID;
    URH_CUDA(ctx, cudaEventRecord(ctx->ev_comp[0], ctx->stream));
    URH_CUDA(ctx, cudaStreamWaitEvent(ctx->copy_stream[0], ctx->ev_comp[0], 0));
    return demod_center_digitize_impl(ctx, d_iq_scratch, dtype, n, has_halo, noise_mag, mod_type, tolerance, samples_per_symbol, max_size,
                                      d_qad_out, true, global_offset, n_total, center, center_state, k, h_iq,
                                      chunk_samples > 0 ? chunk_samples : ((int64_t)1 << 24));
}

extern "C" int urh_shard_demod_center_digitize(urh_ctx* ctx, const void* d_iq, int dtype, int64_t n, int has_halo, float noise_mag,
                                               int mod_type, uint16_t tolerance, uint32_t samples_per_symbol, int64_t max_size,
                                               float* d_qad_out, int64_t global_offset, int64_t n_total, double* center,
                                               int* center_state, int64_t* k) {
    return demod_center_digitize_impl(ctx, d_iq, dtype, n, has_halo, noise_mag, mod_type, tolerance, samples_per_symbol, max_size, d_qad_out,
                                      true, global_offset, n_total, center, center_state, k);
}

extern "C" int urh_afp_demod_stream(urh_ctx* ctx, const void* h_iq, int dtype, int64_t n, float noise_mag, int mod_type, int64_t chunk_samples,
                                    int ring, float* h_qad) {
    if (!h_iq || !h_qad) return URH_ERR_INVALID;
    URH_CHECK(stream_check(ctx, n, ring, mod_type, dtype, true));
    urh_arena_reset(ctx);
    const StreamSizes z = stream_sizes(n, dtype, 0, chunk_samples, ring, URH_STREAM_ENTRY_AFP_DEMOD);
    StreamRing R;
    URH_CHECK(R.init(ctx, ring, z.ring_bytes));
    char* d_src = R.mem;
    float* d_qad = (float*)(R.mem + ring * r256(z.src_slot));
    const UrhDemodParams dp = make_demod_params(noise_mag, mod_type, dtype);
    UrhClassify cls;
    memset(&cls, 0, sizeof(cls));
    return stream_run(ctx, n, z.cs, R, (const char*)h_iq, urh_iq_bytes(dtype), true, d_src, r256(z.src_slot), h_qad, d_qad,
                      [&](int64_t, int64_t s0, int64_t s1, int s) {
                          return stream_dense_iq<false>(ctx, dtype, mod_type, d_src, r256(z.src_slot), n, dp, d_qad + s * z.cs - s0, cls, 0,
                                                        nullptr, s0, s1, s);
                      });
}

extern "C" int urh_grab_pulse_lens_stream(urh_ctx* ctx, const float* qad, int qad_on_device, int64_t n, float center, uint16_t tolerance,
                                          int mod_type, uint32_t samples_per_symbol, uint8_t bits_per_symbol, float center_spacing,
                                          int64_t chunk_samples, int ring, int64_t* k) {
    if (!k || !qad) return URH_ERR_INVALID;
    *k = 0;
    ctx->pulses_k = 0;
    URH_CHECK(stream_check(ctx, n, ring, mod_type, 0, false));
    urh_arena_reset(ctx);
    UrhClassify cls;
    URH_CHECK(fill_classify(ctx, &cls, mod_type, center, bits_per_symbol, center_spacing));
    const StreamSizes z = stream_sizes(n, 0, tolerance, chunk_samples, ring,
                                       URH_STREAM_ENTRY_GRAB_PULSE_LENS | (qad_on_device ? URH_STREAM_QAD_ON_DEVICE : 0));
    StreamRing R;
    URH_CHECK(R.init(ctx, ring, z.ring_bytes));
    StreamDigitizer dz;
    URH_CHECK(dz.init(ctx, n, z.cs, tolerance, mod_type == URH_MOD_ASK, samples_per_symbol));
    char* d_src = R.mem;
    URH_CHECK(stream_run(ctx, n, z.cs, R, qad_on_device ? nullptr : (const char*)qad, 4, false, d_src, r256(z.src_slot), nullptr, nullptr,
                         [&](int64_t, int64_t s0, int64_t s1, int s) {
                             const float* x = qad_on_device ? qad + s0 : (const float*)(d_src + s * r256(z.src_slot) + URH_STREAM_PAD);
                             URH_CHECK(stream_dense_qad(ctx, x, s0, s1, cls, dz));
                             return dz.finish(ctx, s0, s1);
                         }));
    *k = dz.rows;
    return URH_OK;
}

extern "C" int urh_demod_digitize_stream(urh_ctx* ctx, const void* h_iq, int dtype, int64_t n, float noise_mag, int mod_type, float center,
                                         uint16_t tolerance, uint32_t samples_per_symbol, uint8_t bits_per_symbol, float center_spacing,
                                         int64_t chunk_samples, int ring, float* h_qad_out, int64_t* k) {
    if (!k || !h_iq) return URH_ERR_INVALID;
    *k = 0;
    ctx->pulses_k = 0;
    URH_CHECK(stream_check(ctx, n, ring, mod_type, dtype, true));
    urh_arena_reset(ctx);
    UrhClassify cls;
    URH_CHECK(fill_classify(ctx, &cls, mod_type, center, bits_per_symbol, center_spacing));
    const UrhDemodParams dp = make_demod_params(noise_mag, mod_type, dtype);
    const StreamSizes z = stream_sizes(n, dtype, tolerance, chunk_samples, ring,
                                       URH_STREAM_ENTRY_DEMOD_DIGITIZE | (h_qad_out ? URH_STREAM_QAD_OUT : 0));
    StreamRing R;
    URH_CHECK(R.init(ctx, ring, z.ring_bytes));
    StreamDigitizer dz;
    URH_CHECK(dz.init(ctx, n, z.cs, tolerance, mod_type == URH_MOD_ASK, samples_per_symbol));
    char* d_src = R.mem;
    float* d_qad = h_qad_out ? (float*)(R.mem + ring * r256(z.src_slot)) : nullptr;
    URH_CHECK(stream_run(ctx, n, z.cs, R, (const char*)h_iq, urh_iq_bytes(dtype), true, d_src, r256(z.src_slot), h_qad_out, d_qad,
                         [&](int64_t, int64_t s0, int64_t s1, int s) {
                             URH_CHECK(stream_dense_iq<true>(ctx, dtype, mod_type, d_src, r256(z.src_slot), n, dp,
                                                             d_qad ? d_qad + s * z.cs - s0 : nullptr, cls, tolerance, &dz, s0, s1, s));
                             return dz.finish(ctx, s0, s1);
                         }));
    *k = dz.rows;
    return URH_OK;
}

extern "C" int urh_demod_center_digitize_stream(urh_ctx* ctx, const void* h_iq, int dtype, int64_t n, float noise_mag, int mod_type,
                                                uint16_t tolerance, uint32_t samples_per_symbol, int64_t max_size, int64_t chunk_samples,
                                                int ring, float* d_qad_out, float* h_qad_out, double* center, int* center_state,
                                                int64_t* kept, int64_t* k) {
    if (!h_iq || !d_qad_out || !kept) return URH_ERR_INVALID;
    URH_CHECK(stream_check(ctx, n, ring, mod_type, dtype, true));
    StreamCenter sc;
    sc.ring = ring; sc.chunk_samples = chunk_samples; sc.h_iq = h_iq; sc.h_qad = h_qad_out; sc.kept = kept;
    return demod_center_digitize_impl(ctx, nullptr, dtype, n, 0, noise_mag, mod_type, tolerance, samples_per_symbol, max_size, d_qad_out,
                                      false, 0, n, center, center_state, k, nullptr, 0, &sc);
}

extern "C" int urh_afp_demod_psk_stream(urh_ctx* ctx, const void* h_iq, int dtype, int64_t n, float noise_mag, int mod_order,
                                        float costas_loop_bandwidth, int64_t chunk_samples, int ring, float* h_qad) {
    if (!h_iq || !h_qad) return URH_ERR_INVALID;
    URH_CHECK(psk_stream_check(ctx, n, ring, dtype));
    urh_arena_reset(ctx);
    const StreamSizes z = stream_sizes(n, dtype, 0, chunk_samples, ring, URH_STREAM_ENTRY_AFP_DEMOD | psk_entry_flags(mod_order));
    StreamRing R;
    URH_CHECK(R.init(ctx, ring, z.ring_bytes));
    const int64_t slot = r256(z.src_slot);
    char* d_src = R.mem;
    float* d_qad = (float*)(R.mem + ring * slot);
    const UrhDemodParams dp = make_demod_params(noise_mag, URH_MOD_PSK, dtype);
    UrhCostasStream cs;
    URH_CHECK(urh_costas_stream_begin(ctx, &cs));
    const UrhArenaMark mark = urh_arena_mark(ctx);
    URH_CHECK(stream_run(ctx, n, z.cs, R, (const char*)h_iq, urh_iq_bytes(dtype), false, d_src, slot, h_qad, d_qad,
                         [&](int64_t c, int64_t s0, int64_t s1, int s) {
                             urh_arena_release(ctx, mark);
                             return urh_costas_stream_chunk(ctx, &cs, c, d_src + s * slot + URH_STREAM_PAD, dtype, s1 - s0, dp.noise_sqrd,
                                                            mod_order, costas_loop_bandwidth, d_qad + s * z.cs);
                         }));
    return urh_costas_stream_end(ctx, &cs);
}

extern "C" int urh_demod_digitize_psk_stream(urh_ctx* ctx, const void* h_iq, int dtype, int64_t n, float noise_mag, float center,
                                             uint16_t tolerance, uint32_t samples_per_symbol, uint8_t bits_per_symbol, float center_spacing,
                                             int64_t chunk_samples, int ring, float* h_qad_out, int64_t* k) {
    if (!k || !h_iq) return URH_ERR_INVALID;
    *k = 0;
    ctx->pulses_k = 0;
    URH_CHECK(psk_stream_check(ctx, n, ring, dtype));
    urh_arena_reset(ctx);
    UrhClassify cls;
    URH_CHECK(fill_classify(ctx, &cls, URH_MOD_PSK, center, bits_per_symbol, center_spacing));
    const int mod_order = 1 << bits_per_symbol;
    const UrhDemodParams dp = make_demod_params(noise_mag, URH_MOD_PSK, dtype);
    const StreamSizes z = stream_sizes(n, dtype, tolerance, chunk_samples, ring,
                                       URH_STREAM_ENTRY_DEMOD_DIGITIZE | (h_qad_out ? URH_STREAM_QAD_OUT : 0) | psk_entry_flags(mod_order));
    StreamRing R;
    URH_CHECK(R.init(ctx, ring, z.ring_bytes));
    const int64_t slot = r256(z.src_slot);
    char* d_src = R.mem;
    float* d_qad = (float*)(R.mem + ring * slot);
    UrhCostasStream cs;
    URH_CHECK(urh_costas_stream_begin(ctx, &cs));
    StreamDigitizer dz;
    URH_CHECK(dz.init(ctx, n, z.cs, tolerance, false, samples_per_symbol));
    URH_CHECK(stream_run(ctx, n, z.cs, R, (const char*)h_iq, urh_iq_bytes(dtype), false, d_src, slot, h_qad_out, d_qad,
                         [&](int64_t c, int64_t s0, int64_t s1, int s) {
                             urh_arena_release(ctx, dz.mark);
                             float* q = d_qad + s * z.cs;
                             URH_CHECK(urh_costas_stream_chunk(ctx, &cs, c, d_src + s * slot + URH_STREAM_PAD, dtype, s1 - s0, dp.noise_sqrd,
                                                               mod_order, 0.1f, q));
                             URH_CHECK(stream_dense_qad(ctx, q, s0, s1, cls, dz));
                             return dz.finish(ctx, s0, s1);
                         }));
    *k = dz.rows;
    return urh_costas_stream_end(ctx, &cs);
}

struct UrhShardState {
    UrhCandidates cand;
    UrhFireState fs;
    int16_t* d_prev;
};
static UrhShardState* shard_state(urh_ctx* ctx) {
    if (!ctx->shard_state) ctx->shard_state = calloc(1, sizeof(UrhShardState));
    return (UrhShardState*)ctx->shard_state;
}

extern "C" int urh_shard_candidates(urh_ctx* ctx, int carry_valid, int carry_cls, int64_t carry_len, int64_t global_offset,
                                    int64_t* count, const int64_t** d_pos, const int16_t** d_cls, int* last_cand_cls) {
    if (!ctx->shard_tiles) URH_FAIL(ctx, URH_ERR_INVALID, "urh_shard_dense must precede urh_shard_candidates");
    UrhShardCarry in;
    in.valid = carry_valid; in.cls = carry_cls; in.len = carry_len;
    UrhShardState* S = shard_state(ctx);
    URH_CHECK(urh_collect_candidates_shard(ctx, ctx->shard_n, ctx->shard_tol, (const UrhTileSummary*)ctx->shard_tiles,
                                           (const uint32_t*)ctx->shard_staging, ctx->shard_cap, in, global_offset, &S->cand));
    *count = S->cand.count;
    if (d_pos) *d_pos = S->cand.pos;
    if (d_cls) *d_cls = S->cand.cls;
    if (last_cand_cls) {
        *last_cand_cls = 0;
        if (S->cand.count > 0) {
            int16_t v = 0;
            URH_CUDA(ctx, cudaMemcpyAsync(&v, S->cand.cls + S->cand.count - 1, sizeof(v), cudaMemcpyDeviceToHost, ctx->stream));
            URH_CUDA(ctx, cudaStreamSynchronize(ctx->stream));
            *last_cand_cls = v;
        }
    }
    ctx->shard_tiles = nullptr;
    return URH_OK;
}

extern "C" int urh_fetch_candidates(urh_ctx* ctx, int64_t* h_pos, int16_t* h_cls, int64_t count) {
    UrhShardState* S = shard_state(ctx);
    if (count < 0 || count > S->cand.count) URH_FAIL(ctx, URH_ERR_INVALID, "fetch_candidates: count exceeds the table");
    if (count == 0) return URH_OK;
    URH_CUDA(ctx, cudaMemcpyAsync(h_pos, S->cand.pos, (size_t)count * sizeof(int64_t), cudaMemcpyDeviceToHost, ctx->stream));
    URH_CUDA(ctx, cudaMemcpyAsync(h_cls, S->cand.cls, (size_t)count * sizeof(int16_t), cudaMemcpyDeviceToHost, ctx->stream));
    URH_CUDA(ctx, cudaStreamSynchronize(ctx->stream));
    return URH_OK;
}

extern "C" int urh_shard_fire(urh_ctx* ctx, int prev_cls, int64_t* fired, int64_t* last_fired_pos) {
    UrhShardState* S = shard_state(ctx);
    URH_CHECK(urh_arena(ctx, 8, &S->d_prev));
    const int16_t v = (int16_t)prev_cls;
    URH_CUDA(ctx, cudaMemcpyAsync(S->d_prev, &v, sizeof(v), cudaMemcpyHostToDevice, ctx->stream));
    URH_CUDA(ctx, cudaStreamSynchronize(ctx->stream));
    URH_CHECK(urh_fire_stage(ctx, S->cand, S->d_prev, &S->fs, last_fired_pos));
    *fired = S->fs.F;
    return URH_OK;
}

extern "C" int urh_shard_rows(urh_ctx* ctx, int64_t n_total, uint16_t tolerance, int mod_type, uint32_t samples_per_symbol,
                              int64_t prev_fired_pos, int emit_tail, int64_t* k) {
    UrhShardState* S = shard_state(ctx);
    return urh_rows_stage(ctx, S->fs, n_total, tolerance, mod_type == URH_MOD_ASK, samples_per_symbol, prev_fired_pos, emit_tail != 0, k);
}

extern "C" int urh_pulses_from_table(urh_ctx* ctx, const int64_t* d_pos, const int16_t* d_cls, int64_t count, int64_t n_total,
                                     uint16_t tolerance, int mod_type, uint32_t samples_per_symbol, int init_cls, int64_t* k) {
    urh_arena_reset(ctx);
    int16_t* d_init;
    URH_CHECK(urh_arena(ctx, 8, &d_init));
    const int16_t v = (int16_t)init_cls;
    URH_CUDA(ctx, cudaMemcpyAsync(d_init, &v, sizeof(v), cudaMemcpyHostToDevice, ctx->stream));
    URH_CUDA(ctx, cudaStreamSynchronize(ctx->stream));
    UrhCandidates cand;
    cand.count = count;
    cand.pos = (int64_t*)d_pos;
    cand.cls = (int16_t*)d_cls;
    cand.last_cls = 0;
    cand.last_len = 0;
    return urh_pulses_from_candidates(ctx, n_total, tolerance, mod_type == URH_MOD_ASK, samples_per_symbol, cand, d_init, k);
}

extern "C" int urh_fetch_pulses(urh_ctx* ctx, int64_t* h_rows, int64_t k) {
    if (k < 0 || k > ctx->pulses_k) URH_FAIL(ctx, URH_ERR_INVALID, "fetch_pulses: k=%lld exceeds last result %lld", (long long)k, (long long)ctx->pulses_k);
    if (k == 0) return URH_OK;
    URH_CUDA(ctx, cudaMemcpyAsync(h_rows, ctx->pulses, (size_t)k * 2 * sizeof(int64_t), cudaMemcpyDeviceToHost, ctx->stream));
    URH_CUDA(ctx, cudaStreamSynchronize(ctx->stream));
    return URH_OK;
}

extern "C" int urh_pulses_device_ptr(urh_ctx* ctx, const int64_t** d_rows, int64_t* k) {
    if (d_rows) *d_rows = ctx->pulses;
    if (k) *k = ctx->pulses_k;
    return URH_OK;
}


__global__ void k_selftest_div(uint64_t seed, int64_t count, unsigned long long* mismatches, unsigned long long* tested) {
    const int64_t stride = (int64_t)gridDim.x * blockDim.x;
    unsigned long long bad = 0, ok = 0;
    for (int64_t i = (int64_t)blockIdx.x * blockDim.x + threadIdx.x; i < count; i += stride) {
        uint64_t h = seed + (uint64_t)i * 0x9E3779B97F4A7C15ull;
        h = (h ^ (h >> 30)) * 0xBF58476D1CE4E5B9ull;
        h = (h ^ (h >> 27)) * 0x94D049BB133111EBull;
        h ^= h >> 31;
        uint64_t g = h * 0xD6E8FEB86659FD93ull + 0x632BE59BD9B4E019ull;
        g ^= g >> 29;
        const uint32_t span = URH_DIVWIN_HI - URH_DIVWIN_LO;
        uint32_t ea = URH_DIVWIN_LO + (uint32_t)((h >> 40) % span), eb = URH_DIVWIN_LO + (uint32_t)((g >> 40) % span);
        uint32_t ma = (uint32_t)h & 0x7fffff, mb = (uint32_t)g & 0x7fffff;
        if ((i & 15) == 1) ma = 0;
        if ((i & 15) == 2) mb = 0;
        if ((i & 15) == 3) { ma = 0x7fffff; }
        if ((i & 15) == 4) { mb = 0x7fffff; }
        if ((i & 15) == 5) { eb = ea; }
        float a0 = __uint_as_float((ea << 23) | ma), b0 = __uint_as_float((eb << 23) | mb);
        float a1 = __uint_as_float(((URH_DIVWIN_LO + (uint32_t)((g >> 12) % span)) << 23) | ((uint32_t)(h >> 9) & 0x7fffff));
        float b1 = __uint_as_float(((URH_DIVWIN_LO + (uint32_t)((h >> 12) % span)) << 23) | ((uint32_t)(g >> 9) & 0x7fffff));
        if ((i & 15) == 6) { a1 = __uint_as_float((URH_DIVWIN_LO << 23)); b1 = __uint_as_float(((URH_DIVWIN_HI - 1) << 23) | 0x7fffff); }
        if ((i & 15) == 8) { b1 = __uint_as_float((URH_DIVWIN_LO << 23)); a1 = __uint_as_float(((URH_DIVWIN_HI - 1) << 23) | 0x7fffff); }
        if ((i & 63) == 7) a1 = 0.0f;
        const float2 q = urh_div2_window(make_float2(a0, a1), make_float2(b0, b1));
        const float r0 = __fdiv_rn(a0, b0), r1 = __fdiv_rn(a1, b1);
        bad += (__float_as_uint(q.x) != __float_as_uint(r0)) + (__float_as_uint(q.y) != __float_as_uint(r1));
        ok += 2;
    }
    atomicAdd(mismatches, bad);
    atomicAdd(tested, ok);
}

extern "C" int urh_selftest_packed_div(urh_ctx* ctx, uint64_t seed, int64_t count, int64_t* mismatches, int64_t* tested) {
    urh_arena_reset(ctx);
    unsigned long long* d;
    URH_CHECK(urh_arena(ctx, 2, &d));
    URH_CUDA(ctx, cudaMemsetAsync(d, 0, 16, ctx->stream));
    URH_LAUNCH(ctx, k_selftest_div, (unsigned)(ctx->sm_count * 8), 256, 0, seed, count, d, d + 1);
    int64_t h[2];
    URH_CHECK(urh_read_i64(ctx, (const int64_t*)d, 2, h));
    *mismatches = h[0];
    *tested = h[1];
    return URH_OK;
}
```

### urh_b200/csrc/finish.cu

```cuda
#include "sparse.cuh"
#include "tilescan.cuh"

#include <limits.h>

#define CLS_NONE INT_MIN

struct __align__(16) CandAgg {
    int64_t cnt;
    int32_t last_cls;
    int32_t pad;
};
struct CandOp {
    __device__ __forceinline__ CandAgg operator()(const CandAgg& a, const CandAgg& b) const {
        CandAgg r;
        r.cnt = a.cnt + b.cnt;
        r.last_cls = (b.last_cls != CLS_NONE) ? b.last_cls : a.last_cls;
        r.pad = 0;
        return r;
    }
};
struct __align__(16) FireAgg {
    int64_t fired;
    int64_t last_pos;
};
struct FireOp {
    __device__ __forceinline__ FireAgg operator()(const FireAgg& a, const FireAgg& b) const {
        FireAgg r;
        r.fired = a.fired + b.fired;
        r.last_pos = (b.last_pos >= 0) ? b.last_pos : a.last_pos;
        return r;
    }
};

struct ScanRunCarry {
    const UrhTileSummary* tiles;
    int64_t n;
    RunCarry* carry;
    __device__ __forceinline__ RunCarry load(int64_t t) const {
        const int64_t rem = n - t * URH_TILE;
        const int tile_len = rem < URH_TILE ? (int)rem : URH_TILE;
        const UrhTileSummary s = tiles[t];
        RunCarry r;
        r.len = s.tail_len;
        r.cls = s.last_cls;
        r.flags = (s.head_len == tile_len) ? 1 : 0;
        return r;
    }
    __device__ __forceinline__ void post(int64_t t, const RunCarry& excl, const RunCarry&) const { carry[t] = excl; }
};

struct ScanCandidates {
    const UrhTileSummary* tiles;
    const uint32_t* staging;
    int stage_cap;
    const RunCarry* carry;
    const RunCarry* xcarry;
    int tol;
    int32_t* head_rel;
    int32_t* prev_cls;
    __device__ __forceinline__ CandAgg load(int64_t t) const {
        const UrhTileSummary s = tiles[t];
        RunCarry c = carry[t];
        if (xcarry) c = RunCarryOp()(*xcarry, c);
        int64_t start_len = 0;
        if (!(c.flags & 2) && c.cls == s.first_cls) start_len = c.len;
        int32_t rel = -1;
        if (start_len <= tol && (int64_t)tol < start_len + s.head_len) rel = (int32_t)(tol - start_len);
        head_rel[t] = rel;
        CandAgg r;
        r.cnt = (int64_t)s.ncand + (rel >= 0 ? 1 : 0);
        r.last_cls = CLS_NONE;
        if (s.ncand > 0) r.last_cls = (int32_t)(staging[t * (int64_t)stage_cap + s.ncand - 1] & 0xffffu) - 1;
        else if (rel >= 0) r.last_cls = s.first_cls;
        r.pad = 0;
        return r;
    }
    __device__ __forceinline__ void post(int64_t t, const CandAgg& excl, const CandAgg&) const { prev_cls[t] = excl.last_cls; }
};

struct ScanFirings {
    const UrhTileSummary* tiles;
    const uint32_t* staging;
    int stage_cap;
    const int32_t* head_rel;
    const int32_t* prev_cls;
    const int16_t* d_prev0;
    int64_t global_offset;
    int64_t* row_off;
    int64_t* prev_fired;
    __device__ __forceinline__ FireAgg load(int64_t t) const {
        const UrhTileSummary s = tiles[t];
        int prev = prev_cls[t];
        if (prev == CLS_NONE) prev = *d_prev0;
        const int64_t base = t * URH_TILE + global_offset;
        FireAgg r;
        r.fired = 0;
        r.last_pos = -1;
        const int32_t rel = head_rel[t];
        if (rel >= 0) {
            const int c = s.first_cls;
            if (c != prev) { r.fired++; r.last_pos = base + rel; }
            prev = c;
        }
        const uint32_t* st = staging + t * (int64_t)stage_cap;
        for (int j = 0; j < s.ncand; j++) {
            const uint32_t v = st[j];
            const int c = (int)(v & 0xffffu) - 1;
            if (c != prev) { r.fired++; r.last_pos = base + (v >> 16); }
            prev = c;
        }
        return r;
    }
    __device__ __forceinline__ void post(int64_t t, const FireAgg& excl, const FireAgg&) const {
        row_off[t] = excl.fired;
        prev_fired[t] = excl.last_pos;
    }
};

__global__ void __launch_bounds__(256) k_finish_rows(const UrhTileSummary* __restrict__ tiles, const uint32_t* __restrict__ staging,
                                                    int stage_cap, const int32_t* __restrict__ head_rel, const int32_t* __restrict__ prev_cls,
                                                    const int16_t* __restrict__ d_prev0, const int64_t* __restrict__ row_off,
                                                    const int64_t* __restrict__ prev_fired, const int64_t* __restrict__ d_xprev_fired,
                                                    int64_t ntiles, int64_t global_offset, int64_t n_total, int tol, int is_ask, int64_t sps,
                                                    int emit_tail, int64_t row_base, int64_t* __restrict__ out, int64_t cap_rows,
                                                    int64_t* __restrict__ d_out) {
    const int64_t t = (int64_t)blockIdx.x * blockDim.x + threadIdx.x;
    if (t >= ntiles) return;
    const UrhTileSummary s = tiles[t];
    int prev = prev_cls[t];
    if (prev == CLS_NONE) prev = *d_prev0;
    int64_t pp = prev_fired[t];
    if (pp < 0) pp = *d_xprev_fired;
    int64_t idx = row_off[t];
    const int64_t base = t * URH_TILE + global_offset;
    auto fire = [&](int64_t p, int c) {
        if (c != prev) {
            const int64_t rec = (pp >= 0) ? (p - pp) : (p + 1 - tol);
            int64_t st = prev;
            if (is_ask && st == -1 && rec < sps) st = 0;
            if (idx < cap_rows) *((longlong2*)out + idx) = make_longlong2(st, rec);
            idx++;
            pp = p;
        }
        prev = c;
    };
    const int32_t rel = head_rel[t];
    if (rel >= 0) fire(base + rel, s.first_cls);
    const uint32_t* st = staging + t * (int64_t)stage_cap;
    for (int j = 0; j < s.ncand; j++) {
        const uint32_t v = st[j];
        fire(base + (v >> 16), (int)(v & 0xffffu) - 1);
    }
    if (t == ntiles - 1) {
        const int64_t fired = idx;
        if (emit_tail && (is_ask || row_base + fired < n_total)) {
            if (idx < cap_rows) *((longlong2*)out + idx) = make_longlong2(prev, (pp >= 0) ? (n_total - 1 - pp) : (n_total - tol));
            idx++;
        }
        d_out[0] = idx;
        d_out[1] = fired;
    }
}

struct ScanMergeRows {
    const int64_t* raw;
    int64_t rows;
    int64_t n_total;
    int has_tail;
    int64_t* out;
    int64_t* d_k;
    const int64_t* prev_last;
    int64_t row_base;
    __device__ __forceinline__ int64_t load(int64_t r) const {
        if (r == 0) return (prev_last && raw[0] == *prev_last) ? 0 : 1;
        return raw[2 * r] != raw[2 * r - 2] ? 1 : 0;
    }
    __device__ __forceinline__ void post(int64_t r, const int64_t& excl, const int64_t& head) const {
        const bool is_tail = has_tail && r == rows - 1;
        if (is_tail && row_base + excl >= n_total) {
            *d_k = excl;
            return;
        }
        const int64_t o = excl + head - 1;
        if (head) out[2 * o] = raw[2 * r];
        atomicAdd((unsigned long long*)&out[2 * o + 1], (unsigned long long)raw[2 * r + 1]);
        if (r == rows - 1) *d_k = o + 1;
    }
};
struct AddI64 {
    __device__ __forceinline__ int64_t operator()(int64_t a, int64_t b) const { return a + b; }
};

__global__ void k_pack_stage1(const int16_t* __restrict__ d_init, const RunCarry* __restrict__ total, int64_t* __restrict__ msg) {
    memcpy(msg, total, sizeof(RunCarry));
    msg[2] = *d_init;
    msg[3] = 0;
}
__global__ void k_fold_carry(const int64_t* __restrict__ all, int rank, RunCarry* __restrict__ xcarry) {
    RunCarry acc;
    acc.len = 0; acc.cls = 0; acc.flags = 2 | 1;
    for (int q = 0; q < rank; q++) {
        RunCarry c;
        memcpy(&c, all + 4 * q, sizeof(c));
        acc = RunCarryOp()(acc, c);
    }
    if (rank == 0) acc.flags = 2;
    else acc.flags &= ~1;
    *xcarry = acc;
}
__global__ void k_fold_prev_cls(const int64_t* __restrict__ all, int rank, const int64_t* __restrict__ stage1, int16_t* __restrict__ prev0) {
    int v = (int)stage1[2];
    for (int q = 0; q < rank; q++) {
        CandAgg c;
        memcpy(&c, all + 2 * q, sizeof(c));
        if (c.last_cls != CLS_NONE) v = c.last_cls;
    }
    *prev0 = (int16_t)v;
}
__global__ void k_fold_prev_fired(const int64_t* __restrict__ all, int rank, int64_t* __restrict__ xprev) {
    int64_t v = -1;
    for (int q = 0; q < rank; q++) {
        FireAgg c;
        memcpy(&c, all + 2 * q, sizeof(c));
        if (c.last_pos >= 0) v = c.last_pos;
    }
    *xprev = v;
}

__global__ void k_chain_start(const int16_t* __restrict__ d_init, UrhChain* __restrict__ chain) {
    chain->run.len = 0; chain->run.cls = 0; chain->run.flags = 2 | 1;
    chain->prev_fired = -1;
    chain->last_state = INT64_MIN;
    chain->prev_cls = *d_init;
}
__global__ void k_chain_advance(UrhChain* __restrict__ chain, const RunCarry* __restrict__ tot_run, const CandAgg* __restrict__ tot_cand,
                                const FireAgg* __restrict__ tot_fire) {
    chain->run = RunCarryOp()(chain->run, *tot_run);
    if (tot_cand->last_cls != CLS_NONE) chain->prev_cls = (int16_t)tot_cand->last_cls;
    if (tot_fire->last_pos >= 0) chain->prev_fired = tot_fire->last_pos;
}
__global__ void k_chain_last_row(UrhChain* __restrict__ chain, const int64_t* __restrict__ table, int64_t rows) {
    if (rows > 0) chain->last_state = table[2 * (rows - 1)];
}

int urh_coll_allgather(urh_ctx* ctx, const void* d_send, void* d_recv, size_t bytes_per_rank);
extern "C" int urh_p2p_check(urh_ctx* ctx);

struct FinishShard {
    int rank, world;
    int64_t global_offset;
    int64_t n_total;
    int emit_tail;
    UrhChain* chain;
    int64_t row_base, rows_cap;
};

static int finish_tiles(urh_ctx* ctx, int64_t n, int tol, bool is_ask, uint32_t sps, const UrhTileSummary* tiles, const uint32_t* staging,
                        int stage_cap, const int16_t* d_init, const FinishShard& sh, int64_t* k) {
    const int64_t ntiles = urh_div_up(n, URH_TILE);
    const bool sharded = sh.world > 1;
    UrhChain* chain = sh.chain;
    RunCarry* carry;
    int32_t *head_rel, *prev_cls;
    int64_t *row_off, *prev_fired, *d_small;
    URH_CHECK(urh_arena(ctx, (size_t)ntiles, &carry));
    URH_CHECK(urh_arena(ctx, (size_t)ntiles, &head_rel));
    URH_CHECK(urh_arena(ctx, (size_t)ntiles, &prev_cls));
    URH_CHECK(urh_arena(ctx, (size_t)ntiles, &row_off));
    URH_CHECK(urh_arena(ctx, (size_t)ntiles, &prev_fired));
    URH_CHECK(urh_arena(ctx, (size_t)(32 + 8 * (sharded ? sh.world : 0)), &d_small));
    URH_CUDA(ctx, cudaMemsetAsync(d_small, 0xff, 4 * sizeof(int64_t), ctx->stream));
    RunCarry* d_tot_run = (RunCarry*)(d_small + 4);
    CandAgg* d_tot_cand = (CandAgg*)(d_small + 6);
    FireAgg* d_tot_fire = (FireAgg*)(d_small + 8);
    RunCarry* d_xcarry = (RunCarry*)(d_small + 10);
    int16_t* d_prev0 = (int16_t*)(d_small + 12);
    int64_t* d_xprev = d_small + 13;
    int64_t* d_msg1 = d_small + 16;
    int64_t* d_all1 = d_small + 32;
    int64_t* d_all2 = d_all1 + 4 * (sharded ? sh.world : 0);
    int64_t* d_all3 = d_all2 + 2 * (sharded ? sh.world : 0);

    if (chain && sh.global_offset == 0) URH_LAUNCH(ctx, k_chain_start, 1, 1, 0, d_init, chain);
    RunCarry rc_ident;
    rc_ident.len = 0; rc_ident.cls = 0; rc_ident.flags = 2 | 1;
    ScanRunCarry fa;
    fa.tiles = tiles; fa.n = n; fa.carry = carry;
    URH_CHECK((urhts::scan<RunCarry, RunCarryOp, ScanRunCarry>(ctx, ntiles, rc_ident, RunCarryOp(), fa, d_tot_run)));
    if (sharded) {
        URH_LAUNCH(ctx, k_pack_stage1, 1, 1, 0, d_init, (const RunCarry*)d_tot_run, d_msg1);
        URH_TL_MARK(ctx, "x4 run carry: enter");
        URH_CHECK(urh_coll_allgather(ctx, d_msg1, d_all1, 4 * sizeof(int64_t)));
        URH_TL_MARK(ctx, "x4 run carry: done");
        URH_LAUNCH(ctx, k_fold_carry, 1, 1, 0, (const int64_t*)d_all1, sh.rank, d_xcarry);
    }
    ScanCandidates fb;
    fb.tiles = tiles; fb.staging = staging; fb.stage_cap = stage_cap; fb.carry = carry;
    fb.xcarry = sharded ? d_xcarry : (chain ? &chain->run : nullptr);
    fb.tol = tol; fb.head_rel = head_rel; fb.prev_cls = prev_cls;
    CandAgg ca_ident;
    ca_ident.cnt = 0; ca_ident.last_cls = CLS_NONE; ca_ident.pad = 0;
    URH_CHECK((urhts::scan<CandAgg, CandOp, ScanCandidates>(ctx, ntiles, ca_ident, CandOp(), fb, d_tot_cand)));
    const int16_t* prev0 = chain ? &chain->prev_cls : d_init;
    if (sharded) {
        URH_TL_MARK(ctx, "x5 candidates: enter");
        URH_CHECK(urh_coll_allgather(ctx, d_tot_cand, d_all2, sizeof(CandAgg)));
        URH_TL_MARK(ctx, "x5 candidates: done");
        URH_LAUNCH(ctx, k_fold_prev_cls, 1, 1, 0, (const int64_t*)d_all2, sh.rank, (const int64_t*)d_all1, d_prev0);
        prev0 = d_prev0;
    }
    ScanFirings fc;
    fc.tiles = tiles; fc.staging = staging; fc.stage_cap = stage_cap; fc.head_rel = head_rel; fc.prev_cls = prev_cls; fc.d_prev0 = prev0;
    fc.global_offset = sh.global_offset; fc.row_off = row_off; fc.prev_fired = prev_fired;
    FireAgg fi_ident;
    fi_ident.fired = 0; fi_ident.last_pos = -1;
    URH_CHECK((urhts::scan<FireAgg, FireOp, ScanFirings, 4>(ctx, ntiles, fi_ident, FireOp(), fc, d_tot_fire)));
    const int64_t* xprev = chain ? &chain->prev_fired : d_small + 2;
    if (sharded) {
        URH_TL_MARK(ctx, "x6 firings: enter");
        URH_CHECK(urh_coll_allgather(ctx, d_tot_fire, d_all3, sizeof(FireAgg)));
        URH_TL_MARK(ctx, "x6 firings: done");
        URH_LAUNCH(ctx, k_fold_prev_fired, 1, 1, 0, (const int64_t*)d_all3, sh.rank, d_xprev);
        xprev = d_xprev;
    }

    int64_t cap_rows = (int64_t)ctx->pulses_cap_rows;
    const int64_t guess = n / 64 + 1024;
    if (!chain && cap_rows < guess) {
        URH_CHECK(urh_ensure_pulses(ctx, (size_t)guess));
        cap_rows = (int64_t)ctx->pulses_cap_rows;
    }
    const int64_t row_base = chain ? sh.row_base : 0;
    int64_t* raw = ctx->pulses + 2 * row_base;
    int64_t raw_cap = chain ? sh.rows_cap : cap_rows;
    if (is_ask) URH_CHECK(urh_arena(ctx, (size_t)raw_cap * 2, &raw));
    int64_t got[2] = {0, 0};
    for (int attempt = 0; attempt < 2; attempt++) {
        URH_LAUNCH(ctx, k_finish_rows, (unsigned)urh_div_up(ntiles, 256), 256, 0, tiles, staging, stage_cap, (const int32_t*)head_rel,
                   (const int32_t*)prev_cls, prev0, (const int64_t*)row_off, (const int64_t*)prev_fired, xprev, ntiles, sh.global_offset,
                   sh.n_total, tol, is_ask ? 1 : 0, (int64_t)sps, sh.emit_tail, row_base, raw, raw_cap, d_small);
        if (sharded && attempt == 0) URH_TL_MARK(ctx, "rows written");
        URH_CHECK(urh_read_i64(ctx, d_small, 2, got));
        if (sharded) URH_CHECK(urh_p2p_check(ctx));
        if (got[0] <= raw_cap) break;
        if (attempt == 1 || chain) URH_FAIL(ctx, URH_ERR_CUDA, "finish_tiles: row buffer overflow after regrowth");
        if (is_ask) {
            URH_CHECK(urh_arena(ctx, (size_t)got[0] * 2, &raw));
            raw_cap = got[0];
        } else {
            URH_CHECK(urh_ensure_pulses(ctx, (size_t)got[0]));
            raw = ctx->pulses;
            raw_cap = (int64_t)ctx->pulses_cap_rows;
        }
    }
    if (chain) URH_LAUNCH(ctx, k_chain_advance, 1, 1, 0, chain, (const RunCarry*)d_tot_run, (const CandAgg*)d_tot_cand, (const FireAgg*)d_tot_fire);
    int64_t K = got[0];
    if (is_ask && K > 0) {
        if (!chain) URH_CHECK(urh_ensure_pulses(ctx, (size_t)K));
        int64_t* out = ctx->pulses + 2 * row_base;
        URH_CUDA(ctx, cudaMemsetAsync(out, 0, (size_t)K * 2 * sizeof(int64_t), ctx->stream));
        ScanMergeRows fm;
        fm.raw = raw; fm.rows = K; fm.n_total = sh.n_total; fm.has_tail = (sh.emit_tail && K > got[1]) ? 1 : 0; fm.out = out;
        fm.d_k = d_small;
        fm.prev_last = (chain && row_base > 0) ? &chain->last_state : nullptr;
        fm.row_base = row_base;
        URH_CHECK((urhts::scan<int64_t, AddI64, ScanMergeRows>(ctx, K, (int64_t)0, AddI64(), fm, (int64_t*)nullptr)));
        URH_CHECK(urh_read_i64(ctx, d_small, 1, &K));
        if (chain) URH_LAUNCH(ctx, k_chain_last_row, 1, 1, 0, chain, (const int64_t*)ctx->pulses, row_base + K);
    }
    ctx->pulses_k = row_base + K;
    *k = K;
    return URH_OK;
}

int urh_finish_chunk(urh_ctx* ctx, int64_t n, int tol, bool is_ask, uint32_t sps, const UrhTileSummary* tiles, const uint32_t* staging,
                     int stage_cap, const int16_t* d_init, UrhChain* chain, int64_t global_offset, int64_t n_total, int64_t row_base,
                     int64_t rows_cap, int64_t* k) {
    FinishShard sh;
    sh.rank = 0; sh.world = 1; sh.global_offset = global_offset; sh.n_total = n_total;
    sh.emit_tail = (global_offset + n == n_total) ? 1 : 0;
    sh.chain = chain; sh.row_base = row_base; sh.rows_cap = rows_cap;
    return finish_tiles(ctx, n, tol, is_ask, sps, tiles, staging, stage_cap, d_init, sh, k);
}

int urh_finish_local(urh_ctx* ctx, int64_t n, int tol, bool is_ask, uint32_t sps, const UrhTileSummary* tiles, const uint32_t* staging,
                     int stage_cap, const int16_t* d_init, int64_t* k) {
    FinishShard sh;
    sh.rank = 0; sh.world = 1; sh.global_offset = 0; sh.n_total = n; sh.emit_tail = 1;
    sh.chain = nullptr; sh.row_base = 0; sh.rows_cap = 0;
    return finish_tiles(ctx, n, tol, is_ask, sps, tiles, staging, stage_cap, d_init, sh, k);
}

int urh_finish_shard(urh_ctx* ctx, int64_t n, int tol, bool is_ask, uint32_t sps, const UrhTileSummary* tiles, const uint32_t* staging,
                     int stage_cap, const int16_t* d_init, int64_t global_offset, int64_t n_total, int64_t* k) {
    FinishShard sh;
    sh.rank = ctx->nccl_rank; sh.world = ctx->nccl_world; sh.global_offset = global_offset; sh.n_total = n_total;
    sh.emit_tail = (ctx->nccl_rank == ctx->nccl_world - 1) ? 1 : 0;
    sh.chain = nullptr; sh.row_base = 0; sh.rows_cap = 0;
    return finish_tiles(ctx, n, tol, is_ask, sps, tiles, staging, stage_cap, d_init, sh, k);
}
```

### urh_b200/csrc/stats.cu

```cuda
#include "dense_f32.cuh"
#include "scan.cuh"
#include "sparse.cuh"

#include <math.h>

template <int DT>
__device__ __forceinline__ double urh_magnitude(const void* iq, int64_t i) {
    typedef typename UrhElem<DT>::type E;
    const E* p = (const E*)iq + 2 * i;
    if (DT == URH_DT_F32) {
        const float re = (float)p[0], im = (float)p[1];
        return (double)__fsqrt_rn(__fadd_rn(__fmul_rn(re, re), __fmul_rn(im, im)));
    } else {
        const uint32_t re = (uint32_t)(int32_t)p[0], im = (uint32_t)(int32_t)p[1];
        const int32_t ssum = (int32_t)(re * re + im * im);
        return sqrt((double)ssum);
    }
}

template <int DT>
__global__ void k_magnitudes(const void* __restrict__ iq, int64_t n, double* __restrict__ out) {
    const int64_t stride = (int64_t)gridDim.x * blockDim.x;
    for (int64_t i = (int64_t)blockIdx.x * blockDim.x + threadIdx.x; i < n; i += stride) out[i] = urh_magnitude<DT>(iq, i);
}

#define URH_DISPATCH_DT(dtype, KERNEL_CALL)                         \
    switch (dtype) {                                                \
        case URH_DT_I8: { constexpr int DT = URH_DT_I8; KERNEL_CALL; } break;   \
        case URH_DT_U8: { constexpr int DT = URH_DT_U8; KERNEL_CALL; } break;   \
        case URH_DT_I16: { constexpr int DT = URH_DT_I16; KERNEL_CALL; } break; \
        case URH_DT_U16: { constexpr int DT = URH_DT_U16; KERNEL_CALL; } break; \
        case URH_DT_F32: { constexpr int DT = URH_DT_F32; KERNEL_CALL; } break; \
        default: URH_FAIL(ctx, URH_ERR_DTYPE, "Unsupported dtype");  \
    }

extern "C" int urh_get_magnitudes(urh_ctx* ctx, const void* d_iq, int dtype, int64_t n, double* d_out) {
    if (n <= 0) return URH_OK;
    const unsigned grid = (unsigned)min((int64_t)ctx->sm_count * 16, urh_div_up(n, 256));
    URH_DISPATCH_DT(dtype, URH_LAUNCH(ctx, k_magnitudes<DT>, grid, 256, 0, d_iq, n, d_out));
    return URH_OK;
}

#define STAT_BLOCK 256
#define STAT_SLICES 64

template <typename LOADER>
__global__ void __launch_bounds__(STAT_BLOCK) k_chunk_partial(LOADER ld, int64_t n, int64_t cs, int nchunks,
                                                              double* __restrict__ psum, double* __restrict__ pmax) {
    const int chunk = blockIdx.x / STAT_SLICES, slice = blockIdx.x % STAT_SLICES;
    const int64_t c0 = n - (int64_t)(chunk + 1) * cs;
    const int64_t per = urh_div_up(cs, STAT_SLICES);
    const int64_t s0 = c0 + (int64_t)slice * per;
    const int64_t s1 = min(s0 + per, c0 + cs);
    double sum = 0.0, mx = -1.0;
    for (int64_t i = s0 + threadIdx.x; i < s1; i += STAT_BLOCK) {
        const double m = ld(i);
        sum += m;
        mx = fmax(mx, m);
    }
    __shared__ double s_sum[STAT_BLOCK], s_max[STAT_BLOCK];
    s_sum[threadIdx.x] = sum;
    s_max[threadIdx.x] = mx;
    __syncthreads();
    for (int off = STAT_BLOCK / 2; off > 0; off >>= 1) {
        if (threadIdx.x < off) {
            s_sum[threadIdx.x] += s_sum[threadIdx.x + off];
            s_max[threadIdx.x] = fmax(s_max[threadIdx.x], s_max[threadIdx.x + off]);
        }
        __syncthreads();
    }
    if (threadIdx.x == 0) {
        psum[blockIdx.x] = s_sum[0];
        pmax[blockIdx.x] = s_max[0];
    }
}

__global__ void k_chunk_final(const double* __restrict__ psum, const double* __restrict__ pmax, int nchunks,
                              double* __restrict__ sum, double* __restrict__ mx) {
    const int c = blockIdx.x * blockDim.x + threadIdx.x;
    if (c >= nchunks) return;
    double s = 0.0, m = -1.0;
    for (int j = 0; j < STAT_SLICES; j++) {
        s += psum[c * STAT_SLICES + j];
        m = fmax(m, pmax[c * STAT_SLICES + j]);
    }
    sum[c] = s;
    mx[c] = m;
}

template <int DT>
struct LoadMagIQ {
    const void* iq;
    __device__ __forceinline__ double operator()(int64_t i) const { return urh_magnitude<DT>(iq, i); }
};
template <typename T>
struct LoadReal {
    const T* x;
    __device__ __forceinline__ double operator()(int64_t i) const { return (double)x[i]; }
};

template <typename LOADER>
static int chunk_stats(urh_ctx* ctx, LOADER ld, int64_t n, int64_t cs, int nchunks, double* h_sum, double* h_max) {
    urh_arena_reset(ctx);
    double *psum, *pmax, *sum, *mx;
    URH_CHECK(urh_arena(ctx, (size_t)nchunks * STAT_SLICES, &psum));
    URH_CHECK(urh_arena(ctx, (size_t)nchunks * STAT_SLICES, &pmax));
    URH_CHECK(urh_arena(ctx, (size_t)nchunks, &sum));
    URH_CHECK(urh_arena(ctx, (size_t)nchunks, &mx));
    URH_LAUNCH(ctx, (k_chunk_partial<LOADER>), (unsigned)(nchunks * STAT_SLICES), STAT_BLOCK, 0, ld, n, cs, nchunks, psum, pmax);
    URH_LAUNCH(ctx, k_chunk_final, (unsigned)urh_div_up(nchunks, 128), 128, 0, psum, pmax, nchunks, sum, mx);
    URH_CUDA(ctx, cudaMemcpyAsync(h_sum, sum, nchunks * sizeof(double), cudaMemcpyDeviceToHost, ctx->stream));
    URH_CUDA(ctx, cudaMemcpyAsync(h_max, mx, nchunks * sizeof(double), cudaMemcpyDeviceToHost, ctx->stream));
    URH_CUDA(ctx, cudaStreamSynchronize(ctx->stream));
    return URH_OK;
}

extern "C" int urh_noise_chunk_stats_iq(urh_ctx* ctx, const void* d_iq, int dtype, int64_t n, int64_t chunksize,
                                        int nchunks, double* h_sum, double* h_max) {
    if (nchunks <= 0 || chunksize <= 0 || (int64_t)nchunks * chunksize > n) URH_FAIL(ctx, URH_ERR_INVALID, "bad chunking");
    URH_DISPATCH_DT(dtype, { LoadMagIQ<DT> ld; ld.iq = d_iq; URH_CHECK(chunk_stats(ctx, ld, n, chunksize, nchunks, h_sum, h_max)); });
    return URH_OK;
}
extern "C" int urh_noise_chunk_stats(urh_ctx* ctx, const void* d_mags, int is_f64, int64_t n, int64_t chunksize, int nchunks,
                                     double* h_sum, double* h_max) {
    if (nchunks <= 0 || chunksize <= 0 || (int64_t)nchunks * chunksize > n) URH_FAIL(ctx, URH_ERR_INVALID, "bad chunking");
    if (is_f64) {
        LoadReal<double> ld; ld.x = (const double*)d_mags;
        return chunk_stats(ctx, ld, n, chunksize, nchunks, h_sum, h_max);
    }
    LoadReal<float> ld; ld.x = (const float*)d_mags;
    return chunk_stats(ctx, ld, n, chunksize, nchunks, h_sum, h_max);
}

template <typename SRC, typename T>
static int run_table(urh_ctx* ctx, const T* d_x, int64_t n, float thr, int tol, int64_t** h_pos, int16_t** h_cls,
                     int64_t* count, int64_t* h_last) {
    urh_arena_reset(ctx);
    UrhClassify cls;
    memset(&cls, 0, sizeof(cls));
    cls.noise_value = 0.0f;
    cls.order = 2;
    cls.thr[0] = thr;
    const int64_t ntiles = urh_div_up(n, URH_TILE);
    const int cap = URH_TILE / (tol + 1) + 2;
    UrhTileSummary* tiles;
    uint32_t* staging;
    URH_CHECK(urh_arena(ctx, (size_t)ntiles, &tiles));
    URH_CHECK(urh_arena(ctx, (size_t)ntiles * cap, &staging));
    const unsigned grid = (unsigned)urh_div_up(ntiles, URH_WARPS_PER_BLOCK);
    const int vec_in = (((uintptr_t)d_x % (2 * sizeof(T))) == 0) ? 1 : 0;
    URH_LAUNCH(ctx, (k_dense_f32<SRC, T>), grid, URH_WARPS_PER_BLOCK * 32, 0, d_x, n, vec_in, cls, tol, tiles, staging, cap,
               (int16_t*)nullptr, 0);
    UrhCandidates cand;
    URH_CHECK(urh_collect_candidates(ctx, n, tol, tiles, staging, cap, &cand));
    *count = cand.count;
    h_last[0] = cand.last_cls;
    h_last[1] = cand.last_len;
    *h_pos = nullptr;
    *h_cls = nullptr;
    if (cand.count > 0) {
        *h_pos = (int64_t*)malloc((size_t)cand.count * sizeof(int64_t));
        *h_cls = (int16_t*)malloc((size_t)cand.count * sizeof(int16_t));
        URH_CUDA(ctx, cudaMemcpyAsync(*h_pos, cand.pos, (size_t)cand.count * sizeof(int64_t), cudaMemcpyDeviceToHost, ctx->stream));
        URH_CUDA(ctx, cudaMemcpyAsync(*h_cls, cand.cls, (size_t)cand.count * sizeof(int16_t), cudaMemcpyDeviceToHost, ctx->stream));
        URH_CUDA(ctx, cudaStreamSynchronize(ctx->stream));
    }
    return URH_OK;
}

extern "C" int urh_segments_from_runs(const int64_t* h_pos, const int16_t* h_cls, int64_t count, int first_above, int last_cls,
                                      int64_t last_len, int64_t n, int64_t* h_segments, int64_t cap, int64_t* k) {
    int state = first_above ? 1 : 0;
    int64_t start = 0, m = 0;
    for (int64_t j = 0; j < count; j++) {
        if (h_cls[j] == state) continue;
        const int64_t p = h_pos[j];
        if (state == 1) {
            if (m < cap) { h_segments[2 * m] = start; h_segments[2 * m + 1] = p - 10; }
            m++;
            state = 0;
        } else {
            start = p - 10;
            state = 1;
        }
    }
    if (state == 1) {
        const int64_t conseq_below = (last_cls == 0) ? last_len : 0;
        if (start < n - conseq_below) {
            if (m < cap) { h_segments[2 * m] = start; h_segments[2 * m + 1] = n - conseq_below; }
            m++;
        }
    }
    *k = m;
    return URH_OK;
}

extern "C" int urh_segment_shard_pass(urh_ctx* ctx, const void* d_mags, int is_f64, int64_t n, float noise_threshold, int64_t* h_summary) {
    if (n <= 0) URH_FAIL(ctx, URH_ERR_INVALID, "empty shard");
    urh_arena_reset(ctx);
    UrhClassify cls;
    memset(&cls, 0, sizeof(cls));
    cls.noise_value = 0.0f;
    cls.order = 2;
    cls.thr[0] = noise_threshold;
    const int tol = 9;
    const int64_t ntiles = urh_div_up(n, URH_TILE);
    const int cap = URH_TILE / (tol + 1) + 2;
    UrhTileSummary* tiles;
    uint32_t* staging;
    URH_CHECK(urh_arena(ctx, (size_t)ntiles, &tiles));
    URH_CHECK(urh_arena(ctx, (size_t)ntiles * cap, &staging));
    const unsigned grid = (unsigned)urh_div_up(ntiles, URH_WARPS_PER_BLOCK);
    double f0 = 0.0;
    if (is_f64) {
        const int vec_in = (((uintptr_t)d_mags % 16) == 0) ? 1 : 0;
        URH_LAUNCH(ctx, (k_dense_f32<SrcAbove, double>), grid, URH_WARPS_PER_BLOCK * 32, 0, (const double*)d_mags, n, vec_in, cls, tol, tiles,
                   staging, cap, (int16_t*)nullptr, 0);
        URH_CUDA(ctx, cudaMemcpyAsync(&f0, d_mags, sizeof(double), cudaMemcpyDeviceToHost, ctx->stream));
    } else {
        const int vec_in = (((uintptr_t)d_mags % 8) == 0) ? 1 : 0;
        URH_LAUNCH(ctx, (k_dense_f32<SrcAbove, float>), grid, URH_WARPS_PER_BLOCK * 32, 0, (const float*)d_mags, n, vec_in, cls, tol, tiles,
                   staging, cap, (int16_t*)nullptr, 0);
        float f32 = 0.f;
        URH_CUDA(ctx, cudaMemcpyAsync(&f32, d_mags, sizeof(float), cudaMemcpyDeviceToHost, ctx->stream));
        URH_CUDA(ctx, cudaStreamSynchronize(ctx->stream));
        f0 = (double)f32;
    }
    ctx->shard_tiles = tiles;
    ctx->shard_staging = staging;
    ctx->shard_cap = cap;
    ctx->shard_n = n;
    ctx->shard_tol = tol;
    URH_CHECK(urh_shard_run_total(ctx, n, tiles, h_summary));
    h_summary[3] = (is_f64 ? (f0 > (double)noise_threshold) : ((float)f0 > noise_threshold)) ? 1 : 0;
    return URH_OK;
}

extern "C" int urh_segment_messages(urh_ctx* ctx, const void* d_mags, int is_f64, int64_t n, float noise_threshold,
                                    int64_t* h_segments, int64_t cap, int64_t* k) {
    *k = 0;
    if (n <= 0) return URH_OK;
    int64_t* pos = nullptr;
    int16_t* cl = nullptr;
    int64_t count = 0, last[2];
    float first = 0.f;
    if (is_f64) {
        double f0;
        URH_CUDA(ctx, cudaMemcpyAsync(&f0, d_mags, sizeof(double), cudaMemcpyDeviceToHost, ctx->stream));
        URH_CHECK((run_table<SrcAbove, double>(ctx, (const double*)d_mags, n, noise_threshold, 9, &pos, &cl, &count, last)));
        first = (f0 > (double)noise_threshold) ? 1.f : 0.f;
    } else {
        float f0;
        URH_CUDA(ctx, cudaMemcpyAsync(&f0, d_mags, sizeof(float), cudaMemcpyDeviceToHost, ctx->stream));
        URH_CHECK((run_table<SrcAbove, float>(ctx, (const float*)d_mags, n, noise_threshold, 9, &pos, &cl, &count, last)));
        first = (f0 > noise_threshold) ? 1.f : 0.f;
    }
    const int rc = urh_segments_from_runs(pos, cl, count, first > 0.f ? 1 : 0, (int)last[0], last[1], n, h_segments, cap, k);
    free(pos);
    free(cl);
    return rc;
}

extern "C" int urh_plateau_lengths(urh_ctx* ctx, const float* d_rect, int64_t n, float center, int percentage,
                                   uint64_t* h_out, int64_t cap, int64_t* k) {
    *k = 0;
    if (n <= 0) return URH_OK;
    int64_t* pos = nullptr;
    int16_t* cl = nullptr;
    int64_t count = 0, last[2];
    URH_CHECK((run_table<SrcCenter, float>(ctx, d_rect, n, center, 0, &pos, &cl, &count, last)));
    const uint64_t limit = (uint64_t)percentage * (uint64_t)n / 100;
    uint64_t sum = 0;
    int64_t m = 0;
    for (int64_t j = 1; j < count; j++) {
        if (sum >= limit) break;
        const uint64_t len = (uint64_t)(pos[j] - pos[j - 1]);
        if (m < cap) h_out[m] = len;
        m++;
        sum += len;
    }
    if (limit == 0) m = 0;
    free(pos);
    free(cl);
    *k = m;
    return URH_OK;
}

__global__ void k_median(const double* __restrict__ x, int64_t n, int k, float* __restrict__ out) {
    const int64_t i = (int64_t)blockIdx.x * blockDim.x + threadIdx.x;
    if (i >= n) return;
    float buf[64];
    int kk = k;
    if (i + kk > n) kk = (int)(n - i);
    for (int j = 0; j < kk; j++) {
        const float v = (float)x[i + j];
        int p = j;
        while (p > 0 && buf[p - 1] > v) { buf[p] = buf[p - 1]; p--; }
        buf[p] = v;
    }
    out[i] = buf[kk / 2];
}

extern "C" int urh_median_filter(urh_ctx* ctx, const double* d_x, int64_t n, unsigned int k, float* d_out) {
    if (n <= 0) return URH_OK;
    if (k == 0 || k > 64) URH_FAIL(ctx, URH_ERR_INVALID, "median_filter: k must be in 1..64");
    URH_LAUNCH(ctx, k_median, (unsigned)urh_div_up(n, 128), 128, 0, d_x, n, (int)k, d_out);
    return URH_OK;
}

__global__ void k_decibel(const float2* __restrict__ x, int64_t count, float* __restrict__ out) {
    const int64_t stride = (int64_t)gridDim.x * blockDim.x;
    for (int64_t i = (int64_t)blockIdx.x * blockDim.x + threadIdx.x; i < count; i += stride) {
        const float2 v = x[i];
        out[i] = __fmul_rn(10.0f, log10f(__fadd_rn(__fmul_rn(v.x, v.x), __fmul_rn(v.y, v.y))));
    }
}

extern "C" int urh_arr2decibel(urh_ctx* ctx, const float* d_complex, int64_t count, float* d_out) {
    if (count <= 0) return URH_OK;
    const unsigned grid = (unsigned)min((int64_t)ctx->sm_count * 16, urh_div_up(count, 256));
    URH_LAUNCH(ctx, k_decibel, grid, 256, 0, (const float2*)d_complex, count, d_out);
    return URH_OK;
}
```

Measured before the change: 171,200.

## Use persistent grid for dense classify, parallelize guess kernel, merge candidate/fire scans

The dense classification kernel becomes a grid-stride persistent kernel sized by occupancy. Each warp skips noise-only or speculatively resolved tiles together via a ballot, so no lane idles on an early return. The threshold-guess kernel is split across many blocks, with a last-block-done reduction and a parallel peak search. The candidate and firing scans in the finish stage are merged into a single fire-span scan with a per-tile precompute kernel, cutting launches and passes. These add complexity through atomic completion counters and restructured scan state.

```diff
diff --git a/urh_b200/csrc/dense_f32.cuh b/urh_b200/csrc/dense_f32.cuh
--- a/urh_b200/csrc/dense_f32.cuh
+++ b/urh_b200/csrc/dense_f32.cuh
@@ -44,32 +44,12 @@
 template <> struct UrhVec2<double> { typedef double2 type; };
 
 template <typename SRC, typename T>
-__global__ void __launch_bounds__(URH_WARPS_PER_BLOCK * 32)
-k_dense_f32(const T* __restrict__ x, int64_t n, int vec_in, const __grid_constant__ UrhClassify cls, int tol,
-            UrhTileSummary* __restrict__ tiles, uint32_t* __restrict__ staging, int stage_cap,
-            int16_t* __restrict__ init_cls, int cls_of_zero, const float* __restrict__ d_thr0 = nullptr,
-            const UrhTileStats* __restrict__ tile_stats = nullptr, const UrhSpec spec = UrhSpec{}) {
-    const float thr0 = d_thr0 ? *d_thr0 : cls.thr[0];
-    if (d_thr0) cls_of_zero = (0.0f <= thr0) ? 0 : 1;
-    const int lane = threadIdx.x & 31;
-    const int64_t tile = (int64_t)blockIdx.x * URH_WARPS_PER_BLOCK + (threadIdx.x >> 5);
+__device__ __forceinline__ void dense_f32_tile(const T* __restrict__ x, int64_t n, int vec_in, const UrhClassify& cls, float thr0, int cls_of_zero,
+                                               int tol, UrhTileSummary* __restrict__ tiles, uint32_t* __restrict__ staging, int stage_cap,
+                                               int16_t* __restrict__ init_cls, const UrhTileStats* __restrict__ tile_stats, int64_t tile, int lane) {
     const int64_t tile_start = tile * URH_TILE;
-    if (tile_start >= n) return;
     const int tile_len = (int)((n - tile_start) < URH_TILE ? (n - tile_start) : URH_TILE);
     const int iters = (tile_len + 63) >> 6;
-    if (tile_stats && tile_stats[tile].all_noise) {
-        if (lane == 0) {
-            UrhTileSummary s;
-            s.first_cls = -1; s.last_cls = -1; s.head_len = tile_len; s.tail_len = tile_len; s.ncand = 0;
-            tiles[tile] = s;
-            if (tile_start == 0 && init_cls) *init_cls = (int16_t)-1;
-        }
-        return;
-    }
-    if (tile >= spec.lo && tile < spec.hi) {
-        if (spec.margin[tile] > fabsf(__fsub_rn(thr0, *spec.tg))) return;
-        if (lane == 0) atomicAdd(spec.redone, 1u);
-    }
     UrhRunTracker rt;
     rt.init(tol, staging + tile * (int64_t)stage_cap);
     if (vec_in && tile_len == URH_TILE) {
@@ -153,3 +133,57 @@
     }
     rt.finish(tile_len, tiles + tile, lane);
 }
+
+template <typename SRC, typename T>
+__global__ void __launch_bounds__(URH_WARPS_PER_BLOCK * 32)
+k_dense_f32(const T* __restrict__ x, int64_t n, int vec_in, const __grid_constant__ UrhClassify cls, int tol,
+            UrhTileSummary* __restrict__ tiles, uint32_t* __restrict__ staging, int stage_cap,
+            int16_t* __restrict__ init_cls, int cls_of_zero, const float* __restrict__ d_thr0 = nullptr,
+            const UrhTileStats* __restrict__ tile_stats = nullptr, const UrhSpec spec = UrhSpec{}) {
+    const float thr0 = d_thr0 ? *d_thr0 : cls.thr[0];
+    if (d_thr0) cls_of_zero = (0.0f <= thr0) ? 0 : 1;
+    const int lane = threadIdx.x & 31;
+    const int64_t ntiles = urh_div_up(n, URH_TILE);
+    const int64_t nw = (int64_t)gridDim.x * URH_WARPS_PER_BLOCK;
+    const int64_t w = (int64_t)blockIdx.x * URH_WARPS_PER_BLOCK + (threadIdx.x >> 5);
+    for (int64_t k0 = 0; k0 * nw + w < ntiles; k0 += 32) {
+        const int64_t tile = (k0 + lane) * nw + w;
+        bool need = false;
+        if (tile < ntiles) {
+            const int64_t tile_start = tile * URH_TILE;
+            const int tile_len = (int)((n - tile_start) < URH_TILE ? (n - tile_start) : URH_TILE);
+            if (tile_stats && tile_stats[tile].all_noise) {
+                UrhTileSummary s;
+                s.first_cls = -1; s.last_cls = -1; s.head_len = tile_len; s.tail_len = tile_len; s.ncand = 0;
+                tiles[tile] = s;
+                if (tile_start == 0 && init_cls) *init_cls = (int16_t)-1;
+            } else if (tile >= spec.lo && tile < spec.hi) {
+                need = !(spec.margin[tile] > fabsf(__fsub_rn(thr0, *spec.tg)));
+                if (need) atomicAdd(spec.redone, 1u);
+            } else {
+                need = true;
+            }
+        }
+        for (uint32_t b = __ballot_sync(URH_FULL_MASK, need); b; b &= b - 1)
+            dense_f32_tile<SRC, T>(x, n, vec_in, cls, thr0, cls_of_zero, tol, tiles, staging, stage_cap, init_cls, tile_stats,
+                                   (k0 + __ffs(b) - 1) * nw + w, lane);
+    }
+}
+
+template <typename SRC, typename T>
+static int urh_launch_dense_f32(urh_ctx* ctx, const T* x, int64_t n, int vec_in, const UrhClassify& cls, int tol, UrhTileSummary* tiles,
+                                uint32_t* staging, int stage_cap, int16_t* init_cls, int cls_of_zero, const float* d_thr0 = nullptr,
+                                const UrhTileStats* tile_stats = nullptr, const UrhSpec spec = UrhSpec{}) {
+    static int per_sm = 0;
+    if (per_sm == 0) {
+        int b = 0;
+        URH_CUDA(ctx, cudaOccupancyMaxActiveBlocksPerMultiprocessor(&b, k_dense_f32<SRC, T>, URH_WARPS_PER_BLOCK * 32, 0));
+        per_sm = b > 0 ? b : 1;
+    }
+    const int64_t want = urh_div_up(urh_div_up(n, URH_TILE), URH_WARPS_PER_BLOCK);
+    const int64_t fit = (int64_t)ctx->sm_count * per_sm;
+    const unsigned grid = (unsigned)(want < fit ? want : fit);
+    URH_LAUNCH(ctx, (k_dense_f32<SRC, T>), grid, URH_WARPS_PER_BLOCK * 32, 0, x, n, vec_in, cls, tol, tiles, staging, stage_cap, init_cls,
+               cls_of_zero, d_thr0, tile_stats, spec);
+    return URH_OK;
+}
diff --git a/urh_b200/csrc/digitize.cu b/urh_b200/csrc/digitize.cu
--- a/urh_b200/csrc/digitize.cu
+++ b/urh_b200/csrc/digitize.cu
@@ -163,57 +163,89 @@
 
 #define URH_GUESS_SAMPLES 16384
 #define URH_GUESS_BINS 128
-#define URH_GUESS_THREADS 1024
+#define URH_GUESS_THREADS 256
+#define URH_GUESS_BLOCKS (URH_GUESS_SAMPLES / URH_GUESS_THREADS)
+struct UrhGuessWs {
+    float* v;
+    float2* range;
+    unsigned int* done;
+};
 __global__ void __launch_bounds__(URH_GUESS_THREADS) k_speculate_guess(const float2* __restrict__ iq, int64_t n, float noise_sqrd, int forced,
-                                                                      float forced_tg, float* __restrict__ d_tg, unsigned int* __restrict__ redone) {
-    constexpr int PER = URH_GUESS_SAMPLES / URH_GUESS_THREADS;
+                                                                      float forced_tg, float* __restrict__ d_tg, unsigned int* __restrict__ redone,
+                                                                      UrhGuessWs ws) {
     __shared__ unsigned int s_hist[URH_GUESS_BINS];
-    __shared__ float s_mn[32], s_mx[32];
+    __shared__ float s_mn[URH_GUESS_THREADS / 32], s_mx[URH_GUESS_THREADS / 32];
+    __shared__ bool s_last, s_peak[URH_GUESS_BINS];
     if (forced) {
-        if (threadIdx.x == 0) { *d_tg = forced_tg; *redone = 0u; }
+        if (blockIdx.x == 0 && threadIdx.x == 0) { *d_tg = forced_tg; *redone = 0u; }
         return;
     }
-    for (int b = threadIdx.x; b < URH_GUESS_BINS; b += blockDim.x) s_hist[b] = 0u;
-    float v[PER];
+    const int k = blockIdx.x * URH_GUESS_THREADS + threadIdx.x;
+    const int64_t i = 1 + (int64_t)k * (n - 1) / URH_GUESS_SAMPLES;
+    const float2 p = iq[i - 1], c = iq[i];
+    float v = NAN;
     float mn = INFINITY, mx = -INFINITY;
-#pragma unroll
-    for (int k = 0; k < PER; k++) {
-        const int64_t i = 1 + (int64_t)(k * URH_GUESS_THREADS + threadIdx.x) * (n - 1) / URH_GUESS_SAMPLES;
-        const float2 p = iq[i - 1], c = iq[i];
-        v[k] = NAN;
-        if (!(c.x * c.x + c.y * c.y <= noise_sqrd)) {
-            v[k] = atan2f(p.x * c.y - p.y * c.x, p.x * c.x + p.y * c.y);
-            mn = fminf(mn, v[k]);
-            mx = fmaxf(mx, v[k]);
-        }
-    }
+    if (!(c.x * c.x + c.y * c.y <= noise_sqrd)) {
+        v = atan2f(p.x * c.y - p.y * c.x, p.x * c.x + p.y * c.y);
+        mn = fminf(mn, v);
+        mx = fmaxf(mx, v);
+    }
+    ws.v[k] = v;
     for (int off = 16; off > 0; off >>= 1) {
         mn = fminf(mn, __shfl_xor_sync(URH_FULL_MASK, mn, off));
         mx = fmaxf(mx, __shfl_xor_sync(URH_FULL_MASK, mx, off));
     }
     if ((threadIdx.x & 31) == 0) { s_mn[threadIdx.x >> 5] = mn; s_mx[threadIdx.x >> 5] = mx; }
     __syncthreads();
+    if (threadIdx.x == 0) {
+        for (int w = 1; w < URH_GUESS_THREADS / 32; w++) { mn = fminf(mn, s_mn[w]); mx = fmaxf(mx, s_mx[w]); }
+        ws.range[blockIdx.x] = make_float2(mn, mx);
+        __threadfence();
+        s_last = atomicAdd(ws.done, 1u) == gridDim.x - 1;
+    }
+    __syncthreads();
+    if (!s_last) return;
+    __threadfence();
+    for (int b = threadIdx.x; b < URH_GUESS_BINS; b += blockDim.x) s_hist[b] = 0u;
     mn = INFINITY; mx = -INFINITY;
-    for (int w = 0; w < URH_GUESS_THREADS / 32; w++) { mn = fminf(mn, s_mn[w]); mx = fmaxf(mx, s_mx[w]); }
+    for (int b = 0; b < URH_GUESS_BLOCKS; b++) {
+        const float2 r = __ldcg(ws.range + b);
+        mn = fminf(mn, r.x);
+        mx = fmaxf(mx, r.y);
+    }
+    __syncthreads();
     const float width = (mx - mn) / URH_GUESS_BINS;
     if (width > 0.0f) {
+        constexpr int PER = URH_GUESS_SAMPLES / 4 / URH_GUESS_THREADS;
+        float4 x[PER];
 #pragma unroll
-        for (int k = 0; k < PER; k++)
-            if (!isnan(v[k])) atomicAdd(&s_hist[min((int)((v[k] - mn) / width), URH_GUESS_BINS - 1)], 1u);
+        for (int q = 0; q < PER; q++) x[q] = __ldcg((const float4*)ws.v + q * URH_GUESS_THREADS + threadIdx.x);
+#pragma unroll
+        for (int q = 0; q < PER; q++) {
+            const float e[4] = {x[q].x, x[q].y, x[q].z, x[q].w};
+#pragma unroll
+            for (int r = 0; r < 4; r++)
+                if (!isnan(e[r])) atomicAdd(&s_hist[min((int)((e[r] - mn) / width), URH_GUESS_BINS - 1)], 1u);
+        }
+    }
+    __syncthreads();
+    constexpr int WINDOW = (int)(0.05 * URH_GUESS_BINS) + 1;
+    for (int b = threadIdx.x; b < URH_GUESS_BINS; b += blockDim.x) {
+        const unsigned int y = s_hist[b];
+        bool peak = y > 0u;
+        for (int d = 1; d < WINDOW && peak; d++)
+            peak = y > (b + d < URH_GUESS_BINS ? s_hist[b + d] : 0u) && y > (b - d >= 0 ? s_hist[b - d] : 0u);
+        s_peak[b] = peak;
     }
     __syncthreads();
     if (threadIdx.x != 0) return;
     *redone = 0u;
     if (!(mn <= mx)) { *d_tg = 0.0f; return; }
     if (!(width > 0.0f)) { *d_tg = mn; return; }
-    constexpr int WINDOW = (int)(0.05 * URH_GUESS_BINS) + 1;
     int top[2] = {-1, -1};
     for (int b = 0; b < URH_GUESS_BINS; b++) {
+        if (!s_peak[b]) continue;
         const unsigned int y = s_hist[b];
-        bool peak = y > 0u;
-        for (int d = 1; d < WINDOW && peak; d++)
-            peak = y > (b + d < URH_GUESS_BINS ? s_hist[b + d] : 0u) && y > (b - d >= 0 ? s_hist[b - d] : 0u);
-        if (!peak) continue;
         if (top[0] < 0 || y > s_hist[top[0]]) { top[1] = top[0]; top[0] = b; }
         else if (top[1] < 0 || y > s_hist[top[1]]) top[1] = b;
     }
@@ -445,15 +477,14 @@
     URH_CHECK(urh_arena(ctx, (size_t)ntiles, &tiles));
     URH_CHECK(urh_arena(ctx, (size_t)ntiles * cap, &staging));
     URH_CHECK(urh_arena(ctx, 8, &d_init));
-    const unsigned grid = (unsigned)urh_div_up(ntiles, URH_WARPS_PER_BLOCK);
     const int vec_in = (((uintptr_t)d_qad % 8) == 0) ? 1 : 0;
     URH_PROF_BEGIN(ctx);
     if (cls.order == 2)
-        URH_LAUNCH(ctx, (k_dense_f32<SrcQad2, float>), grid, URH_WARPS_PER_BLOCK * 32, 0, d_qad, n, vec_in, cls, tol, tiles,
-                   staging, cap, d_init, host_classify(0.0f, cls));
+        URH_CHECK((urh_launch_dense_f32<SrcQad2, float>(ctx, d_qad, n, vec_in, cls, tol, tiles,
+                   staging, cap, d_init, host_classify(0.0f, cls))));
     else
-        URH_LAUNCH(ctx, (k_dense_f32<SrcQad, float>), grid, URH_WARPS_PER_BLOCK * 32, 0, d_qad, n, vec_in, cls, tol, tiles,
-                   staging, cap, d_init, host_classify(0.0f, cls));
+        URH_CHECK((urh_launch_dense_f32<SrcQad, float>(ctx, d_qad, n, vec_in, cls, tol, tiles,
+                   staging, cap, d_init, host_classify(0.0f, cls))));
     URH_PROF_END(ctx);
     return digitize_finish(ctx, n, tol, mod_type == URH_MOD_ASK, samples_per_symbol, tiles, staging, cap, d_init, k);
 }
@@ -557,13 +588,12 @@
     URH_CUDA(ctx, cudaMemsetAsync(d_init, 0, 16, ctx->stream));
     const int vec_in = (((uintptr_t)d_qad % 8) == 0) ? 1 : 0;
     URH_PROF_BEGIN(ctx);
-    const unsigned grid = (unsigned)urh_div_up(ntiles, URH_WARPS_PER_BLOCK);
     if (cls.order == 2)
-        URH_LAUNCH(ctx, (k_dense_f32<SrcQad2, float>), grid, URH_WARPS_PER_BLOCK * 32, 0, d_qad, n, vec_in, cls, tol, tiles, staging, cap,
-                   d_init, host_classify(0.0f, cls));
+        URH_CHECK((urh_launch_dense_f32<SrcQad2, float>(ctx, d_qad, n, vec_in, cls, tol, tiles, staging, cap,
+                   d_init, host_classify(0.0f, cls))));
     else
-        URH_LAUNCH(ctx, (k_dense_f32<SrcQad, float>), grid, URH_WARPS_PER_BLOCK * 32, 0, d_qad, n, vec_in, cls, tol, tiles, staging, cap,
-                   d_init, host_classify(0.0f, cls));
+        URH_CHECK((urh_launch_dense_f32<SrcQad, float>(ctx, d_qad, n, vec_in, cls, tol, tiles, staging, cap,
+                   d_init, host_classify(0.0f, cls))));
     URH_PROF_END(ctx);
     ctx->shard_tiles = tiles;
     ctx->shard_staging = staging;
@@ -861,17 +891,16 @@
 static int stream_dense_qad(urh_ctx* ctx, const float* x, int64_t s0, int64_t s1, const UrhClassify& cls, StreamDigitizer& dz,
                             const float* d_thr0 = nullptr, const UrhTileStats* ts = nullptr) {
     const int64_t nc = s1 - s0;
-    const unsigned grid = (unsigned)urh_div_up(urh_div_up(nc, URH_TILE), URH_WARPS_PER_BLOCK);
     const int vec_in = (((uintptr_t)x % 8) == 0) ? 1 : 0;
     int16_t* init = s0 == 0 ? dz.d_init : nullptr;
     const int c0 = d_thr0 ? 0 : host_classify(0.0f, cls);
     const UrhTileStats* tsc = ts ? ts + s0 / URH_TILE : nullptr;
     if (cls.order == 2)
-        URH_LAUNCH(ctx, (k_dense_f32<SrcQad2, float>), grid, URH_WARPS_PER_BLOCK * 32, 0, x, nc, vec_in, cls, dz.tol, dz.tiles, dz.staging,
-                   dz.cap, init, c0, d_thr0, tsc);
+        URH_CHECK((urh_launch_dense_f32<SrcQad2, float>(ctx, x, nc, vec_in, cls, dz.tol, dz.tiles, dz.staging,
+                   dz.cap, init, c0, d_thr0, tsc)));
     else
-        URH_LAUNCH(ctx, (k_dense_f32<SrcQad, float>), grid, URH_WARPS_PER_BLOCK * 32, 0, x, nc, vec_in, cls, dz.tol, dz.tiles, dz.staging,
-                   dz.cap, init, c0, d_thr0, tsc);
+        URH_CHECK((urh_launch_dense_f32<SrcQad, float>(ctx, x, nc, vec_in, cls, dz.tol, dz.tiles, dz.staging,
+                   dz.cap, init, c0, d_thr0, tsc)));
     return URH_OK;
 }
 
@@ -908,14 +937,13 @@
     const int c0 = host_classify(0.0f, cls);
     if (d_qad_in) {
         const int vec_in = (((uintptr_t)d_qad_in % 8) == 0) ? 1 : 0;
-        const unsigned grid = (unsigned)urh_div_up(ntiles, URH_WARPS_PER_BLOCK);
-        URH_PROF_BEGIN(ctx);
+            URH_PROF_BEGIN(ctx);
         if (cls.order == 2)
-            URH_LAUNCH(ctx, (k_dense_f32<SrcQad2, float>), grid, URH_WARPS_PER_BLOCK * 32, 0, d_qad_in, n, vec_in, cls, tol, tiles, staging, cap,
-                       d_init, c0, (const float*)nullptr);
+            URH_CHECK((urh_launch_dense_f32<SrcQad2, float>(ctx, d_qad_in, n, vec_in, cls, tol, tiles, staging, cap,
+                       d_init, c0, (const float*)nullptr)));
         else
-            URH_LAUNCH(ctx, (k_dense_f32<SrcQad, float>), grid, URH_WARPS_PER_BLOCK * 32, 0, d_qad_in, n, vec_in, cls, tol, tiles, staging, cap,
-                       d_init, c0, (const float*)nullptr);
+            URH_CHECK((urh_launch_dense_f32<SrcQad, float>(ctx, d_qad_in, n, vec_in, cls, tol, tiles, staging, cap,
+                       d_init, c0, (const float*)nullptr)));
         URH_PROF_END(ctx);
     } else {
         const UrhDemodParams dp = make_demod_params(noise_mag, mod_type, dtype);
@@ -1003,9 +1031,14 @@
         URH_CHECK(urh_arena(ctx, 1, &spec.redone));
         URH_CHECK(urh_arena(ctx, (size_t)ntiles, &spec.margin));
         spec.tg = tg;
+        UrhGuessWs gws;
+        URH_CHECK(urh_arena(ctx, URH_GUESS_SAMPLES, &gws.v));
+        URH_CHECK(urh_arena(ctx, URH_GUESS_BLOCKS, &gws.range));
+        URH_CHECK(urh_arena(ctx, 1, &gws.done));
+        URH_CUDA(ctx, cudaMemsetAsync(gws.done, 0, sizeof(unsigned int), ctx->stream));
         const char* forced = getenv("URH_B200_SPECULATE_GUESS");
-        URH_LAUNCH(ctx, k_speculate_guess, 1, URH_GUESS_THREADS, 0, (const float2*)d_iq, n, dp.noise_sqrd, forced ? 1 : 0,
-                   forced ? strtof(forced, nullptr) : 0.0f, tg, spec.redone);
+        URH_LAUNCH(ctx, k_speculate_guess, URH_GUESS_BLOCKS, URH_GUESS_THREADS, 0, (const float2*)d_iq, n, dp.noise_sqrd, forced ? 1 : 0,
+                   forced ? strtof(forced, nullptr) : 0.0f, tg, spec.redone, gws);
     }
     int chunk_no = 0;
     for (int64_t t0 = 0; t0 < (sc ? 0 : ntiles); t0 += chunk_tiles, chunk_no++) {
@@ -1055,8 +1088,8 @@
     } else {
         URH_CUDA(ctx, cudaMemsetAsync(d_init, 0, 16, ctx->stream));
         const int vec_in = (((uintptr_t)d_qad_out % 8) == 0) ? 1 : 0;
-        URH_LAUNCH(ctx, (k_dense_f32<SrcQad2, float>), (unsigned)urh_div_up(ntiles, URH_WARPS_PER_BLOCK), URH_WARPS_PER_BLOCK * 32, 0,
-                   (const float*)d_qad_out, n, vec_in, cls, tol, tiles, staging, cap, d_init, 0, d_centerf, (const UrhTileStats*)ts, spec);
+        URH_CHECK((urh_launch_dense_f32<SrcQad2, float>(ctx, (const float*)d_qad_out, n, vec_in, cls, tol, tiles, staging, cap, d_init, 0,
+                                                        d_centerf, (const UrhTileStats*)ts, spec)));
         URH_CUDA(ctx, cudaMemcpyAsync(ctx->h_mail + 40, d_center, sizeof(double), cudaMemcpyDeviceToHost, ctx->stream));
         URH_CUDA(ctx, cudaMemcpyAsync(ctx->h_mail + 41, d_state, sizeof(int), cudaMemcpyDeviceToHost, ctx->stream));
         URH_CHECK(urh_center_plan_certify_stats(ctx, plan, ctx->h_mail + 42));
diff --git a/urh_b200/csrc/finish.cu b/urh_b200/csrc/finish.cu
--- a/urh_b200/csrc/finish.cu
+++ b/urh_b200/csrc/finish.cu
@@ -5,31 +5,47 @@
 
 #define CLS_NONE INT_MIN
 
-struct __align__(16) CandAgg {
-    int64_t cnt;
+struct __align__(16) FireSpan {
+    int64_t fired;
+    int64_t first_pos;
+    int64_t last_fire;
+    int32_t first_cls;
     int32_t last_cls;
-    int32_t pad;
-};
-struct CandOp {
-    __device__ __forceinline__ CandAgg operator()(const CandAgg& a, const CandAgg& b) const {
-        CandAgg r;
-        r.cnt = a.cnt + b.cnt;
-        r.last_cls = (b.last_cls != CLS_NONE) ? b.last_cls : a.last_cls;
-        r.pad = 0;
+};
+struct FireOp {
+    __device__ __forceinline__ FireSpan operator()(const FireSpan& a, const FireSpan& b) const {
+        if (b.first_cls == CLS_NONE) return a;
+        if (a.first_cls == CLS_NONE) return b;
+        const bool fire = a.last_cls != b.first_cls;
+        FireSpan r;
+        r.fired = a.fired + b.fired + (fire ? 1 : 0);
+        r.first_pos = a.first_pos;
+        r.last_fire = (b.last_fire >= 0) ? b.last_fire : (fire ? b.first_pos : a.last_fire);
+        r.first_cls = a.first_cls;
+        r.last_cls = b.last_cls;
         return r;
     }
 };
-struct __align__(16) FireAgg {
+__device__ __forceinline__ FireSpan fire_empty() {
+    FireSpan r;
+    r.fired = 0; r.first_pos = -1; r.last_fire = -1; r.first_cls = CLS_NONE; r.last_cls = CLS_NONE;
+    return r;
+}
+__device__ __forceinline__ FireSpan fire_seed(int prev_cls, int64_t prev_fired) {
+    FireSpan r;
+    r.fired = 0; r.first_pos = -1; r.last_fire = prev_fired; r.first_cls = prev_cls; r.last_cls = prev_cls;
+    return r;
+}
+struct __align__(8) TileFire {
     int64_t fired;
-    int64_t last_pos;
-};
-struct FireOp {
-    __device__ __forceinline__ FireAgg operator()(const FireAgg& a, const FireAgg& b) const {
-        FireAgg r;
-        r.fired = a.fired + b.fired;
-        r.last_pos = (b.last_pos >= 0) ? b.last_pos : a.last_pos;
-        return r;
-    }
+    int64_t last_fire;
+    int32_t last_cls;
+    int32_t head_rel;
+};
+struct __align__(16) TileFires {
+    uint32_t first, last;
+    int32_t fired;
+    int32_t last_rel;
 };
 
 struct ScanRunCarry {
@@ -49,16 +65,63 @@
     __device__ __forceinline__ void post(int64_t t, const RunCarry& excl, const RunCarry&) const { carry[t] = excl; }
 };
 
-struct ScanCandidates {
+#define FIN_WARPS 8
+#define FIN_ROW 33
+
+__device__ __forceinline__ int64_t shfl_i64(int64_t v, int src) {
+    return (int64_t)__shfl_sync(URH_FULL_MASK, (unsigned long long)v, src);
+}
+__device__ __forceinline__ void stage_words(const uint32_t* __restrict__ staging, int stage_cap, int64_t t0, int m_lane, uint32_t* s,
+                                            int lane) {
+#pragma unroll
+    for (int i = 0; i < 32; i++) {
+        const int m = __shfl_sync(URH_FULL_MASK, m_lane, i);
+        s[i * FIN_ROW + lane] = (lane < m) ? __ldg(staging + (t0 + i) * (int64_t)stage_cap + lane) : 0u;
+    }
+    __syncwarp();
+}
+__device__ __forceinline__ uint32_t staged_word(const uint32_t* s, const uint32_t* __restrict__ staging, int stage_cap, int64_t t0, int i,
+                                                int j) {
+    return j < 32 ? s[i * FIN_ROW + j] : __ldg(staging + (t0 + i) * (int64_t)stage_cap + j);
+}
+
+__global__ void __launch_bounds__(FIN_WARPS * 32) k_tile_fires(const UrhTileSummary* __restrict__ tiles, const uint32_t* __restrict__ staging,
+                                                             int stage_cap, int64_t ntiles, TileFires* __restrict__ out) {
+    __shared__ uint32_t s_words[FIN_WARPS][32 * FIN_ROW];
+    const int lane = threadIdx.x & 31, warp = threadIdx.x >> 5;
+    const int64_t t0 = ((int64_t)blockIdx.x * FIN_WARPS + warp) * 32;
+    if (t0 >= ntiles) return;
+    const int64_t my = t0 + lane;
+    const int m = (my < ntiles) ? tiles[my].ncand : 0;
+    uint32_t* s = s_words[warp];
+    stage_words(staging, stage_cap, t0, m, s, lane);
+    TileFires r;
+    r.first = r.last = 0u; r.fired = 0; r.last_rel = -1;
+    if (m > 0) {
+        uint32_t prev = s[lane * FIN_ROW];
+        r.first = prev;
+        for (int j = 1; j < m; j++) {
+            const uint32_t w = staged_word(s, staging, stage_cap, t0, lane, j);
+            if ((w ^ prev) & 0xffffu) {
+                r.fired++;
+                r.last_rel = (int)(w >> 16);
+            }
+            prev = w;
+        }
+        r.last = prev;
+    }
+    if (my < ntiles) out[my] = r;
+}
+
+struct ScanFires {
     const UrhTileSummary* tiles;
-    const uint32_t* staging;
-    int stage_cap;
+    const TileFires* fires;
     const RunCarry* carry;
     const RunCarry* xcarry;
     int tol;
-    int32_t* head_rel;
-    int32_t* prev_cls;
-    __device__ __forceinline__ CandAgg load(int64_t t) const {
+    int64_t global_offset;
+    TileFire* tf;
+    __device__ __forceinline__ FireSpan load(int64_t t) const {
         const UrhTileSummary s = tiles[t];
         RunCarry c = carry[t];
         if (xcarry) c = RunCarryOp()(*xcarry, c);
@@ -66,92 +129,111 @@
         if (!(c.flags & 2) && c.cls == s.first_cls) start_len = c.len;
         int32_t rel = -1;
         if (start_len <= tol && (int64_t)tol < start_len + s.head_len) rel = (int32_t)(tol - start_len);
-        head_rel[t] = rel;
-        CandAgg r;
-        r.cnt = (int64_t)s.ncand + (rel >= 0 ? 1 : 0);
-        r.last_cls = CLS_NONE;
-        if (s.ncand > 0) r.last_cls = (int32_t)(staging[t * (int64_t)stage_cap + s.ncand - 1] & 0xffffu) - 1;
-        else if (rel >= 0) r.last_cls = s.first_cls;
-        r.pad = 0;
+        tf[t].head_rel = rel;
+        const int64_t base = t * URH_TILE + global_offset;
+        FireSpan r = fire_empty();
+        if (s.ncand > 0) {
+            const TileFires f = fires[t];
+            r.fired = f.fired;
+            r.first_pos = base + (f.first >> 16);
+            r.last_fire = (f.last_rel >= 0) ? base + f.last_rel : -1;
+            r.first_cls = (int32_t)(f.first & 0xffffu) - 1;
+            r.last_cls = (int32_t)(f.last & 0xffffu) - 1;
+        }
+        if (rel >= 0) {
+            FireSpan h = fire_empty();
+            h.first_pos = base + rel;
+            h.first_cls = h.last_cls = s.first_cls;
+            r = FireOp()(h, r);
+        }
         return r;
     }
-    __device__ __forceinline__ void post(int64_t t, const CandAgg& excl, const CandAgg&) const { prev_cls[t] = excl.last_cls; }
-};
-
-struct ScanFirings {
-    const UrhTileSummary* tiles;
-    const uint32_t* staging;
-    int stage_cap;
-    const int32_t* head_rel;
-    const int32_t* prev_cls;
-    const int16_t* d_prev0;
-    int64_t global_offset;
-    int64_t* row_off;
-    int64_t* prev_fired;
-    __device__ __forceinline__ FireAgg load(int64_t t) const {
-        const UrhTileSummary s = tiles[t];
-        int prev = prev_cls[t];
-        if (prev == CLS_NONE) prev = *d_prev0;
-        const int64_t base = t * URH_TILE + global_offset;
-        FireAgg r;
-        r.fired = 0;
-        r.last_pos = -1;
-        const int32_t rel = head_rel[t];
-        if (rel >= 0) {
-            const int c = s.first_cls;
-            if (c != prev) { r.fired++; r.last_pos = base + rel; }
-            prev = c;
-        }
-        const uint32_t* st = staging + t * (int64_t)stage_cap;
-        for (int j = 0; j < s.ncand; j++) {
-            const uint32_t v = st[j];
-            const int c = (int)(v & 0xffffu) - 1;
-            if (c != prev) { r.fired++; r.last_pos = base + (v >> 16); }
-            prev = c;
-        }
-        return r;
-    }
-    __device__ __forceinline__ void post(int64_t t, const FireAgg& excl, const FireAgg&) const {
-        row_off[t] = excl.fired;
-        prev_fired[t] = excl.last_pos;
-    }
-};
-
-__global__ void __launch_bounds__(256) k_finish_rows(const UrhTileSummary* __restrict__ tiles, const uint32_t* __restrict__ staging,
-                                                    int stage_cap, const int32_t* __restrict__ head_rel, const int32_t* __restrict__ prev_cls,
-                                                    const int16_t* __restrict__ d_prev0, const int64_t* __restrict__ row_off,
-                                                    const int64_t* __restrict__ prev_fired, const int64_t* __restrict__ d_xprev_fired,
-                                                    int64_t ntiles, int64_t global_offset, int64_t n_total, int tol, int is_ask, int64_t sps,
-                                                    int emit_tail, int64_t row_base, int64_t* __restrict__ out, int64_t cap_rows,
-                                                    int64_t* __restrict__ d_out) {
-    const int64_t t = (int64_t)blockIdx.x * blockDim.x + threadIdx.x;
-    if (t >= ntiles) return;
-    const UrhTileSummary s = tiles[t];
-    int prev = prev_cls[t];
-    if (prev == CLS_NONE) prev = *d_prev0;
-    int64_t pp = prev_fired[t];
-    if (pp < 0) pp = *d_xprev_fired;
-    int64_t idx = row_off[t];
-    const int64_t base = t * URH_TILE + global_offset;
-    auto fire = [&](int64_t p, int c) {
-        if (c != prev) {
-            const int64_t rec = (pp >= 0) ? (p - pp) : (p + 1 - tol);
-            int64_t st = prev;
-            if (is_ask && st == -1 && rec < sps) st = 0;
-            if (idx < cap_rows) *((longlong2*)out + idx) = make_longlong2(st, rec);
-            idx++;
-            pp = p;
-        }
-        prev = c;
-    };
-    const int32_t rel = head_rel[t];
-    if (rel >= 0) fire(base + rel, s.first_cls);
-    const uint32_t* st = staging + t * (int64_t)stage_cap;
-    for (int j = 0; j < s.ncand; j++) {
-        const uint32_t v = st[j];
-        fire(base + (v >> 16), (int)(v & 0xffffu) - 1);
-    }
-    if (t == ntiles - 1) {
+    __device__ __forceinline__ void post(int64_t t, const FireSpan& excl, const FireSpan&) const {
+        tf[t].fired = excl.fired;
+        tf[t].last_fire = excl.last_fire;
+        tf[t].last_cls = excl.last_cls;
+    }
+};
+
+__global__ void __launch_bounds__(FIN_WARPS * 32) k_finish_rows(const UrhTileSummary* __restrict__ tiles, const uint32_t* __restrict__ staging,
+                                                              int stage_cap, const TileFire* __restrict__ tf, const FireSpan* __restrict__ tot,
+                                                              const int16_t* __restrict__ seed_cls, const int64_t* __restrict__ seed_fired,
+                                                              int64_t ntiles, int64_t global_offset, int64_t n_total, int tol, int is_ask, int64_t sps,
+                                                              int emit_tail, int64_t row_base, int64_t* __restrict__ out, int64_t cap_rows,
+                                                              int64_t* __restrict__ d_out) {
+    __shared__ uint32_t s_words[FIN_WARPS][32 * FIN_ROW];
+    const int lane = threadIdx.x & 31, warp = threadIdx.x >> 5;
+    const int64_t t0 = ((int64_t)blockIdx.x * FIN_WARPS + warp) * 32;
+    if (t0 >= ntiles) return;
+    const uint32_t lt = (1u << lane) - 1u;
+    const int64_t my = t0 + lane;
+    int m_l = 0, rel_l = -1, fcls_l = 0;
+    if (my < ntiles) {
+        m_l = tiles[my].ncand;
+        fcls_l = tiles[my].first_cls;
+        rel_l = tf[my].head_rel;
+    }
+    int prev;
+    int64_t pp, idx;
+    {
+        const TileFire f = tf[t0];
+        FireSpan ex;
+        ex.fired = f.fired; ex.last_fire = f.last_fire; ex.last_cls = f.last_cls;
+        ex.first_cls = (f.last_cls == CLS_NONE) ? CLS_NONE : tot->first_cls;
+        ex.first_pos = tot->first_pos;
+        const FireSpan e = FireOp()(fire_seed(*seed_cls, *seed_fired), ex);
+        prev = e.last_cls; pp = e.last_fire; idx = e.fired;
+    }
+    uint32_t* s = s_words[warp];
+    stage_words(staging, stage_cap, t0, m_l, s, lane);
+    const int cnt = m_l + (rel_l >= 0 ? 1 : 0);
+    int incl = cnt;
+#pragma unroll
+    for (int off = 1; off < 32; off <<= 1) {
+        const int v = __shfl_up_sync(URH_FULL_MASK, incl, off);
+        if (lane >= off) incl += v;
+    }
+    const int total = __shfl_sync(URH_FULL_MASK, incl, 31);
+    for (int k0 = 0; k0 < total; k0 += 32) {
+        const int k = k0 + lane;
+        const bool valid = k < total;
+        int i = 0;
+#pragma unroll
+        for (int step = 16; step > 0; step >>= 1)
+            if (__shfl_sync(URH_FULL_MASK, incl, i + step - 1) <= k) i += step;
+        const int ti = __shfl_sync(URH_FULL_MASK, incl, i) , ci = __shfl_sync(URH_FULL_MASK, cnt, i);
+        const int rel = __shfl_sync(URH_FULL_MASK, rel_l, i), fcls = __shfl_sync(URH_FULL_MASK, fcls_l, i);
+        const int e = k - (ti - ci);
+        int p = 0, c = CLS_NONE;
+        if (valid) {
+            if (rel >= 0 && e == 0) {
+                p = rel; c = fcls;
+            } else {
+                const uint32_t v = staged_word(s, staging, stage_cap, t0, i, e - (rel >= 0 ? 1 : 0));
+                p = (int)(v >> 16); c = (int)(v & 0xffffu) - 1;
+            }
+        }
+        int pc = __shfl_up_sync(URH_FULL_MASK, c, 1);
+        if (lane == 0) pc = prev;
+        const bool f = valid && c != pc;
+        const uint32_t b = __ballot_sync(URH_FULL_MASK, f);
+        const int64_t gp = (t0 + i) * URH_TILE + global_offset + p;
+        const uint32_t below = b & lt;
+        const int64_t fb = shfl_i64(gp, below ? 31 - __clz(below) : 0);
+        if (f) {
+            const int64_t q = below ? fb : pp;
+            const int64_t rec = (q >= 0) ? (gp - q) : (gp + 1 - tol);
+            int64_t stt = pc;
+            if (is_ask && stt == -1 && rec < sps) stt = 0;
+            const int64_t slot = idx + __popc(below);
+            if (slot < cap_rows) *((longlong2*)out + slot) = make_longlong2(stt, rec);
+        }
+        idx += __popc(b);
+        const int64_t lf = shfl_i64(gp, b ? 31 - __clz(b) : 0);
+        if (b) pp = lf;
+        prev = __shfl_sync(URH_FULL_MASK, c, min(31, total - 1 - k0));
+    }
+    if (t0 + 32 >= ntiles && lane == 0) {
         const int64_t fired = idx;
         if (emit_tail && (is_ask || row_base + fired < n_total)) {
             if (idx < cap_rows) *((longlong2*)out + idx) = make_longlong2(prev, (pp >= 0) ? (n_total - 1 - pp) : (n_total - tol));
@@ -208,23 +290,22 @@
     else acc.flags &= ~1;
     *xcarry = acc;
 }
-__global__ void k_fold_prev_cls(const int64_t* __restrict__ all, int rank, const int64_t* __restrict__ stage1, int16_t* __restrict__ prev0) {
-    int v = (int)stage1[2];
+__device__ __forceinline__ void fire_fold(int16_t& prev_cls, int64_t& prev_fired, const FireSpan& tot) {
+    const FireSpan r = FireOp()(fire_seed(prev_cls, prev_fired), tot);
+    prev_cls = (int16_t)r.last_cls;
+    prev_fired = r.last_fire;
+}
+__global__ void k_fold_fire(const int64_t* __restrict__ all, int rank, const int64_t* __restrict__ stage1, int16_t* __restrict__ prev0,
+                            int64_t* __restrict__ xprev) {
+    int16_t c = (int16_t)stage1[2];
+    int64_t f = -1;
     for (int q = 0; q < rank; q++) {
-        CandAgg c;
-        memcpy(&c, all + 2 * q, sizeof(c));
-        if (c.last_cls != CLS_NONE) v = c.last_cls;
-    }
-    *prev0 = (int16_t)v;
-}
-__global__ void k_fold_prev_fired(const int64_t* __restrict__ all, int rank, int64_t* __restrict__ xprev) {
-    int64_t v = -1;
-    for (int q = 0; q < rank; q++) {
-        FireAgg c;
-        memcpy(&c, all + 2 * q, sizeof(c));
-        if (c.last_pos >= 0) v = c.last_pos;
-    }
-    *xprev = v;
+        FireSpan t;
+        memcpy(&t, all + 4 * q, sizeof(t));
+        fire_fold(c, f, t);
+    }
+    *prev0 = c;
+    *xprev = f;
 }
 
 __global__ void k_chain_start(const int16_t* __restrict__ d_init, UrhChain* __restrict__ chain) {
@@ -233,11 +314,9 @@
     chain->last_state = INT64_MIN;
     chain->prev_cls = *d_init;
 }
-__global__ void k_chain_advance(UrhChain* __restrict__ chain, const RunCarry* __restrict__ tot_run, const CandAgg* __restrict__ tot_cand,
-                                const FireAgg* __restrict__ tot_fire) {
+__global__ void k_chain_advance(UrhChain* __restrict__ chain, const RunCarry* __restrict__ tot_run, const FireSpan* __restrict__ tot_fire) {
     chain->run = RunCarryOp()(chain->run, *tot_run);
-    if (tot_cand->last_cls != CLS_NONE) chain->prev_cls = (int16_t)tot_cand->last_cls;
-    if (tot_fire->last_pos >= 0) chain->prev_fired = tot_fire->last_pos;
+    fire_fold(chain->prev_cls, chain->prev_fired, *tot_fire);
 }
 __global__ void k_chain_last_row(UrhChain* __restrict__ chain, const int64_t* __restrict__ table, int64_t rows) {
     if (rows > 0) chain->last_state = table[2 * (rows - 1)];
@@ -261,27 +340,26 @@
     const bool sharded = sh.world > 1;
     UrhChain* chain = sh.chain;
     RunCarry* carry;
-    int32_t *head_rel, *prev_cls;
-    int64_t *row_off, *prev_fired, *d_small;
+    TileFires* fires;
+    TileFire* tf;
+    int64_t* d_small;
     URH_CHECK(urh_arena(ctx, (size_t)ntiles, &carry));
-    URH_CHECK(urh_arena(ctx, (size_t)ntiles, &head_rel));
-    URH_CHECK(urh_arena(ctx, (size_t)ntiles, &prev_cls));
-    URH_CHECK(urh_arena(ctx, (size_t)ntiles, &row_off));
-    URH_CHECK(urh_arena(ctx, (size_t)ntiles, &prev_fired));
+    URH_CHECK(urh_arena(ctx, (size_t)ntiles, &fires));
+    URH_CHECK(urh_arena(ctx, (size_t)ntiles, &tf));
     URH_CHECK(urh_arena(ctx, (size_t)(32 + 8 * (sharded ? sh.world : 0)), &d_small));
     URH_CUDA(ctx, cudaMemsetAsync(d_small, 0xff, 4 * sizeof(int64_t), ctx->stream));
     RunCarry* d_tot_run = (RunCarry*)(d_small + 4);
-    CandAgg* d_tot_cand = (CandAgg*)(d_small + 6);
-    FireAgg* d_tot_fire = (FireAgg*)(d_small + 8);
-    RunCarry* d_xcarry = (RunCarry*)(d_small + 10);
-    int16_t* d_prev0 = (int16_t*)(d_small + 12);
-    int64_t* d_xprev = d_small + 13;
+    FireSpan* d_tot_fire = (FireSpan*)(d_small + 8);
+    RunCarry* d_xcarry = (RunCarry*)(d_small + 12);
+    int16_t* d_prev0 = (int16_t*)(d_small + 14);
+    int64_t* d_xprev = d_small + 15;
     int64_t* d_msg1 = d_small + 16;
     int64_t* d_all1 = d_small + 32;
     int64_t* d_all2 = d_all1 + 4 * (sharded ? sh.world : 0);
-    int64_t* d_all3 = d_all2 + 2 * (sharded ? sh.world : 0);
 
     if (chain && sh.global_offset == 0) URH_LAUNCH(ctx, k_chain_start, 1, 1, 0, d_init, chain);
+    const unsigned fin_grid = (unsigned)urh_div_up(ntiles, 32 * FIN_WARPS);
+    URH_LAUNCH(ctx, k_tile_fires, fin_grid, FIN_WARPS * 32, 0, tiles, staging, stage_cap, ntiles, fires);
     RunCarry rc_ident;
     rc_ident.len = 0; rc_ident.cls = 0; rc_ident.flags = 2 | 1;
     ScanRunCarry fa;
@@ -294,34 +372,22 @@
         URH_TL_MARK(ctx, "x4 run carry: done");
         URH_LAUNCH(ctx, k_fold_carry, 1, 1, 0, (const int64_t*)d_all1, sh.rank, d_xcarry);
     }
-    ScanCandidates fb;
-    fb.tiles = tiles; fb.staging = staging; fb.stage_cap = stage_cap; fb.carry = carry;
+    ScanFires fb;
+    fb.tiles = tiles; fb.fires = fires; fb.carry = carry;
     fb.xcarry = sharded ? d_xcarry : (chain ? &chain->run : nullptr);
-    fb.tol = tol; fb.head_rel = head_rel; fb.prev_cls = prev_cls;
-    CandAgg ca_ident;
-    ca_ident.cnt = 0; ca_ident.last_cls = CLS_NONE; ca_ident.pad = 0;
-    URH_CHECK((urhts::scan<CandAgg, CandOp, ScanCandidates>(ctx, ntiles, ca_ident, CandOp(), fb, d_tot_cand)));
-    const int16_t* prev0 = chain ? &chain->prev_cls : d_init;
+    fb.tol = tol; fb.global_offset = sh.global_offset; fb.tf = tf;
+    FireSpan fs_ident;
+    fs_ident.fired = 0; fs_ident.first_pos = -1; fs_ident.last_fire = -1; fs_ident.first_cls = CLS_NONE; fs_ident.last_cls = CLS_NONE;
+    URH_CHECK((urhts::scan<FireSpan, FireOp, ScanFires, 4>(ctx, ntiles, fs_ident, FireOp(), fb, d_tot_fire)));
+    const int16_t* seed_cls = chain ? &chain->prev_cls : d_init;
+    const int64_t* seed_fired = chain ? &chain->prev_fired : d_small + 2;
     if (sharded) {
-        URH_TL_MARK(ctx, "x5 candidates: enter");
-        URH_CHECK(urh_coll_allgather(ctx, d_tot_cand, d_all2, sizeof(CandAgg)));
-        URH_TL_MARK(ctx, "x5 candidates: done");
-        URH_LAUNCH(ctx, k_fold_prev_cls, 1, 1, 0, (const int64_t*)d_all2, sh.rank, (const int64_t*)d_all1, d_prev0);
-        prev0 = d_prev0;
-    }
-    ScanFirings fc;
-    fc.tiles = tiles; fc.staging = staging; fc.stage_cap = stage_cap; fc.head_rel = head_rel; fc.prev_cls = prev_cls; fc.d_prev0 = prev0;
-    fc.global_offset = sh.global_offset; fc.row_off = row_off; fc.prev_fired = prev_fired;
-    FireAgg fi_ident;
-    fi_ident.fired = 0; fi_ident.last_pos = -1;
-    URH_CHECK((urhts::scan<FireAgg, FireOp, ScanFirings, 4>(ctx, ntiles, fi_ident, FireOp(), fc, d_tot_fire)));
-    const int64_t* xprev = chain ? &chain->prev_fired : d_small + 2;
-    if (sharded) {
-        URH_TL_MARK(ctx, "x6 firings: enter");
-        URH_CHECK(urh_coll_allgather(ctx, d_tot_fire, d_all3, sizeof(FireAgg)));
-        URH_TL_MARK(ctx, "x6 firings: done");
-        URH_LAUNCH(ctx, k_fold_prev_fired, 1, 1, 0, (const int64_t*)d_all3, sh.rank, d_xprev);
-        xprev = d_xprev;
+        URH_TL_MARK(ctx, "x5 firings: enter");
+        URH_CHECK(urh_coll_allgather(ctx, d_tot_fire, d_all2, sizeof(FireSpan)));
+        URH_TL_MARK(ctx, "x5 firings: done");
+        URH_LAUNCH(ctx, k_fold_fire, 1, 1, 0, (const int64_t*)d_all2, sh.rank, (const int64_t*)d_all1, d_prev0, d_xprev);
+        seed_cls = d_prev0;
+        seed_fired = d_xprev;
     }
 
     int64_t cap_rows = (int64_t)ctx->pulses_cap_rows;
@@ -336,9 +402,9 @@
     if (is_ask) URH_CHECK(urh_arena(ctx, (size_t)raw_cap * 2, &raw));
     int64_t got[2] = {0, 0};
     for (int attempt = 0; attempt < 2; attempt++) {
-        URH_LAUNCH(ctx, k_finish_rows, (unsigned)urh_div_up(ntiles, 256), 256, 0, tiles, staging, stage_cap, (const int32_t*)head_rel,
-                   (const int32_t*)prev_cls, prev0, (const int64_t*)row_off, (const int64_t*)prev_fired, xprev, ntiles, sh.global_offset,
-                   sh.n_total, tol, is_ask ? 1 : 0, (int64_t)sps, sh.emit_tail, row_base, raw, raw_cap, d_small);
+        URH_LAUNCH(ctx, k_finish_rows, fin_grid, FIN_WARPS * 32, 0, tiles, staging, stage_cap, (const TileFire*)tf, (const FireSpan*)d_tot_fire,
+                   seed_cls, seed_fired, ntiles, sh.global_offset, sh.n_total, tol, is_ask ? 1 : 0, (int64_t)sps, sh.emit_tail, row_base, raw,
+                   raw_cap, d_small);
         if (sharded && attempt == 0) URH_TL_MARK(ctx, "rows written");
         URH_CHECK(urh_read_i64(ctx, d_small, 2, got));
         if (sharded) URH_CHECK(urh_p2p_check(ctx));
@@ -353,7 +419,7 @@
             raw_cap = (int64_t)ctx->pulses_cap_rows;
         }
     }
-    if (chain) URH_LAUNCH(ctx, k_chain_advance, 1, 1, 0, chain, (const RunCarry*)d_tot_run, (const CandAgg*)d_tot_cand, (const FireAgg*)d_tot_fire);
+    if (chain) URH_LAUNCH(ctx, k_chain_advance, 1, 1, 0, chain, (const RunCarry*)d_tot_run, (const FireSpan*)d_tot_fire);
     int64_t K = got[0];
     if (is_ask && K > 0) {
         if (!chain) URH_CHECK(urh_ensure_pulses(ctx, (size_t)K));
diff --git a/urh_b200/csrc/stats.cu b/urh_b200/csrc/stats.cu
--- a/urh_b200/csrc/stats.cu
+++ b/urh_b200/csrc/stats.cu
@@ -147,10 +147,9 @@
     uint32_t* staging;
     URH_CHECK(urh_arena(ctx, (size_t)ntiles, &tiles));
     URH_CHECK(urh_arena(ctx, (size_t)ntiles * cap, &staging));
-    const unsigned grid = (unsigned)urh_div_up(ntiles, URH_WARPS_PER_BLOCK);
     const int vec_in = (((uintptr_t)d_x % (2 * sizeof(T))) == 0) ? 1 : 0;
-    URH_LAUNCH(ctx, (k_dense_f32<SRC, T>), grid, URH_WARPS_PER_BLOCK * 32, 0, d_x, n, vec_in, cls, tol, tiles, staging, cap,
-               (int16_t*)nullptr, 0);
+    URH_CHECK((urh_launch_dense_f32<SRC, T>(ctx, d_x, n, vec_in, cls, tol, tiles, staging, cap,
+               (int16_t*)nullptr, 0)));
     UrhCandidates cand;
     URH_CHECK(urh_collect_candidates(ctx, n, tol, tiles, staging, cap, &cand));
     *count = cand.count;
@@ -210,17 +209,16 @@
     uint32_t* staging;
     URH_CHECK(urh_arena(ctx, (size_t)ntiles, &tiles));
     URH_CHECK(urh_arena(ctx, (size_t)ntiles * cap, &staging));
-    const unsigned grid = (unsigned)urh_div_up(ntiles, URH_WARPS_PER_BLOCK);
     double f0 = 0.0;
     if (is_f64) {
         const int vec_in = (((uintptr_t)d_mags % 16) == 0) ? 1 : 0;
-        URH_LAUNCH(ctx, (k_dense_f32<SrcAbove, double>), grid, URH_WARPS_PER_BLOCK * 32, 0, (const double*)d_mags, n, vec_in, cls, tol, tiles,
-                   staging, cap, (int16_t*)nullptr, 0);
+        URH_CHECK((urh_launch_dense_f32<SrcAbove, double>(ctx, (const double*)d_mags, n, vec_in, cls, tol, tiles,
+                   staging, cap, (int16_t*)nullptr, 0)));
         URH_CUDA(ctx, cudaMemcpyAsync(&f0, d_mags, sizeof(double), cudaMemcpyDeviceToHost, ctx->stream));
     } else {
         const int vec_in = (((uintptr_t)d_mags % 8) == 0) ? 1 : 0;
-        URH_LAUNCH(ctx, (k_dense_f32<SrcAbove, float>), grid, URH_WARPS_PER_BLOCK * 32, 0, (const float*)d_mags, n, vec_in, cls, tol, tiles,
-                   staging, cap, (int16_t*)nullptr, 0);
+        URH_CHECK((urh_launch_dense_f32<SrcAbove, float>(ctx, (const float*)d_mags, n, vec_in, cls, tol, tiles,
+                   staging, cap, (int16_t*)nullptr, 0)));
         float f32 = 0.f;
         URH_CUDA(ctx, cudaMemcpyAsync(&f32, d_mags, sizeof(float), cudaMemcpyDeviceToHost, ctx->stream));
         URH_CUDA(ctx, cudaStreamSynchronize(ctx->stream));
```

Measured after the change: 173,600 (median of 6 runs). No clear change (+1.4%).
